# rasd3/TODA

Measured on NVIDIA B200. Metric: frames/s voxelize+VoxelResBackBone8x fwd+bwd, higher is better.
Workload: dtype bf16

## Files before the change

### include/toda_b200.h

```cpp
#ifndef TODA_B200_H
#define TODA_B200_H

#include <stddef.h>
#include <stdint.h>

#ifdef __cplusplus
extern "C" {
#endif

#define TODA_OK 0
#define TODA_ERR_INVALID (-1)
#define TODA_ERR_CUDA (-2)
#define TODA_ERR_WORKSPACE (-3)
#define TODA_ERR_UNSUPPORTED (-4)

#define TODA_ORDER_FIRST_APPEARANCE 0
#define TODA_ORDER_CANONICAL 1

const char *toda_last_error(void);
int toda_version(void);
long long toda_launch_count(void);
int toda_device_info(int *sm_count_host, int *cc_major_host, int *cc_minor_host);

size_t toda_index_bytes(int batch, int D, int H, int W);
int toda_index_insert(void *index, int batch, int D, int H, int W, const int32_t *coords, int n, void *stream);
int toda_index_insert_strided(void *index_out, int batch, int oD, int oH, int oW, const int32_t *in_coords, int n_in,
                              const int *ksize_host, const int *stride_host, const int *pad_host, void *stream);
int toda_index_build(void *index, int batch, int D, int H, int W, int32_t *out_coords, int cap, int32_t *n_out,
                     void *stream);
int toda_index_rows(const void *index, int batch, int D, int H, int W, const int32_t *coords, int n, int32_t *rows,
                    void *stream);
int toda_index_release(void *index, int batch, int D, int H, int W, const int32_t *coords, int n, void *stream);

#define TODA_SELECT_RANGE_XY 0
#define TODA_SELECT_RECT_XY 1
#define TODA_SELECT_SECTOR 2
#define TODA_SELECT_BOXES 3
size_t toda_points_select_workspace_bytes(int n);
int toda_points_select(const float *points, int n, int stride, int x_col, const int32_t *frame_offsets, int batch, int mode,
                       const double *params_host, int invert, int add_batch_col, float *out, int32_t *out_offsets,
                       void *workspace, size_t workspace_bytes, void *stream);

#define TODA_WORLD_FLIP_X 0
#define TODA_WORLD_FLIP_Y 1
#define TODA_WORLD_ROTATE 2
#define TODA_WORLD_SCALE 3
int toda_points_world_transform(const float *points, int n, int stride, int x_col, const int32_t *frame_offsets, int batch,
                                int n_steps, const int *kinds_host, const float *params_host, float *out, void *stream);

size_t toda_voxelize_workspace_bytes(int64_t n_points, int batch, const int *grid_host, int max_points,
                                     int max_voxels);
int toda_voxelize_hard(const float *points, int64_t n_points, int point_stride, int xyz_col, int feat_col,
                       int num_features, const int32_t *frame_offsets, int batch, const float *range_host,
                       const float *vsize_host, const int *grid_host, int max_points, int max_voxels, int order,
                       float *voxels, int32_t *coords, int32_t *num_points, int32_t *voxel_counts, void *workspace,
                       size_t workspace_bytes, void *stream);

int toda_mean_vfe_fwd(const float *voxels, const void *num_points, int num_is_float, int n_voxels, int max_points,
                      int num_features, float *voxel_features, void *stream);
int toda_mean_vfe_bwd(const float *d_voxel_features, const void *num_points, int num_is_float, int n_voxels,
                      int max_points, int num_features, float *d_voxels, void *stream);

int toda_rulebook_subm(const void *index, int batch, int D, int H, int W, const int32_t *coords, int n,
                       const int *ksize_host, int32_t *nbr, void *stream);
int toda_rulebook_sparse(const void *index_in, int iD, int iH, int iW, const void *index_out, int oD, int oH, int oW,
                         int batch, const int32_t *in_coords, int n_in, const int32_t *out_coords, int n_out,
                         const int *ksize_host, const int *stride_host, const int *pad_host, int32_t *nbr_fwd,
                         int32_t *nbr_bwd, void *stream);

size_t toda_parity_order_workspace_bytes(int n);
int toda_parity_order(const int32_t *coords, int n, const int *stride_host, const int *pad_host, int32_t *order,
                      int32_t *pos_of_row, void *workspace, size_t workspace_bytes, void *stream);

#define TODA_CONV_FP32 0
#define TODA_CONV_BF16 1
#define TODA_CONV_BF16X3 2
int toda_weight_repack(const float *w_param, int kvol, int cin, int cout, int transpose, int mirror_k, float *w_out,
                       void *stream);
size_t toda_spconv_fwd_workspace_bytes(int n_in, int cin, int cout, int kvol, int precision);
int toda_table_tile_masks(const int32_t *nbr, int n_out, int kvol, uint32_t *masks, void *stream);
int toda_spconv_uses_tensor_cores(int cin, int cout, int kvol, int precision);
int toda_spconv_wgrad_uses_tensor_cores(int cin, int cout, int kvol, int precision);
int toda_spconv_fwd(const float *x, const void *x_bf16, int n_in, int cin, const int32_t *nbr, int n_out, int kvol,
                    const float *w, int cout, const float *bias, float *y, const int32_t *out_rows,
                    const uint32_t *tile_masks, double *bn_sums, int precision, void *workspace, size_t workspace_bytes,
                    void *stream);
int toda_tile_plan_capacity(int channels);
int toda_table_tile_plan(const int32_t *nbr, int n_out, int kvol, int ngroups, int cap, uint16_t *lidx, int32_t *rows,
                         int32_t *cnt, void *stream);
int toda_spconv_fwd_plan(const float *x, const void *x_bf16, int n_in, int cin, const int32_t *nbr, int n_out, int kvol,
                         const float *w, int cout, const float *bias, const float *addend, float *y,
                         const int32_t *out_rows, const uint32_t *tile_masks, const uint16_t *plan_lidx,
                         const int32_t *plan_rows, const int32_t *plan_cnt, int plan_groups, int plan_cap, double *bn_sums,
                         const void *w_bf16, int precision, void *workspace, size_t workspace_bytes, void *stream);
int toda_weight_kmajor_bf16(const float *w, int kvol, int cin, int cout, void *w_bf16, void *stream);
size_t toda_spconv_wgrad_workspace_bytes(int n_in, int n_out, int kvol, int cin, int cout, int precision);
int toda_spconv_wgrad(const float *x, const void *x_bf16, int n_in, int cin, const int32_t *nbr, int n_out, int kvol,
                      const uint32_t *tile_masks, const float *dy, const void *dy_bf16, int cout, float *dw_param,
                      void *workspace, size_t workspace_bytes, int precision, void *stream);
int toda_spconv_wgrad_row_splits(const uint32_t *tile_masks, int n_out, int kvol, int cin, int cout, int *groups,
                                 int *splits, int32_t *row_begin, void *stream);

size_t toda_bn_workspace_bytes(int channels);
int toda_bn_local_sums(const float *y, const double *epilogue_sums, int n, int channels, double *sums, double *count,
                       void *workspace, size_t workspace_bytes, void *stream);
int toda_bn_eval_coeffs(const float *gamma, const float *beta, const float *running_mean, const float *running_var,
                        float eps, int channels, float *scale, float *shift, void *stream);
int toda_bn_apply(const float *y, int n, int channels, const float *scale, const float *shift, const float *residual,
                  int relu, float *a, void *a_bf16, void *stream);
int toda_bn_apply_sums(const float *y, int n, int channels, const double *sums, const double *count, const float *gamma,
                       const float *beta, float eps, float momentum, float *running_mean, float *running_var, float *scale,
                       float *shift, float *save_mean, float *save_rstd, const float *residual, int relu, float *a,
                       void *a_bf16, void *stream);
int toda_bn_bwd_reduce(const float *da, const float *a, const float *y, int n, int channels, const float *save_mean,
                       const float *save_rstd, int relu, double *red, float *dgamma, float *dbeta, void *workspace,
                       size_t workspace_bytes, void *stream);
int toda_bn_bwd_finish(const float *da, const float *a, const float *y, int n, int channels, const float *gamma,
                       const float *save_mean, const float *save_rstd, int relu, int training, const double *red,
                       const double *count, float *dy, void *dy_bf16, float *dresidual, float *dbias, void *workspace,
                       size_t workspace_bytes, void *stream);
int toda_bn_bwd(const float *da, const float *a, const float *y, int n, int channels, const float *gamma,
                const float *save_mean, const float *save_rstd, int relu, int training, float *dy, void *dy_bf16,
                float *dresidual, float *dgamma, float *dbeta, float *dbias, void *workspace, size_t workspace_bytes,
                void *stream);
int toda_col_sum(const float *dy, int n, int channels, float *out, void *workspace, size_t workspace_bytes,
                 void *stream);

typedef struct {
    const float *x; const void *x_bf16; int n_in, cin; const int32_t *nbr; int n_out, kvol;
    const float *w; const void *w_bf16 ; int cout; const float *bias ;
    const uint32_t *tile_masks ;
    const uint16_t *plan_lidx ; const int32_t *plan_rows; const int32_t *plan_cnt; int plan_groups, plan_cap;
    int precision; void *conv_ws; size_t conv_ws_bytes;
    const float *gamma; const float *beta; float eps, momentum; float *running_mean; float *running_var; int training;
    const float *residual ; int relu;
    float *y; double *sums; float *stats; float *a; void *a_bf16 ;
    void *bn_ws; size_t bn_ws_bytes;
} toda_layer_fwd_args;
typedef struct {
    const float *da; const float *a_mask; const float *y; int n_out, cout; const float *gamma; const float *mean; const float *rstd;
    int relu, training; float *dy; void *dy_bf16 ; float *dres ; float *dgamma; float *dbeta;
    void *bn_ws; size_t bn_ws_bytes;
    const float *x; const void *x_bf16 ; int n_in, cin, kvol;
    int need_dx; const int32_t *dgrad_nbr; const float *wt; const void *wt_bf16 ;
    const int32_t *dgrad_out_rows ; const uint32_t *dgrad_masks ;
    const uint16_t *dplan_lidx ; const int32_t *dplan_rows; const int32_t *dplan_cnt; int dplan_groups, dplan_cap;
    const float *addend ; float *dx;
    int need_dw; const int32_t *nbr_fwd; const uint32_t *fwd_masks ; float *dw;
    void *wgrad_ws; size_t wgrad_ws_bytes;
    int need_db; float *db;
    int precision; void *conv_ws; size_t conv_ws_bytes;
} toda_layer_bwd_args;
int toda_layer_fwd(const toda_layer_fwd_args *args, void *stream);
int toda_layer_bwd(const toda_layer_bwd_args *args, void *stream);
int toda_layer_fwd_stats(const toda_layer_fwd_args *args, double *local_sums, void *stream);
int toda_layer_fwd_apply(const toda_layer_fwd_args *args, const double *global_sums, void *stream);
int toda_layer_bwd_reduce(const toda_layer_bwd_args *args, double *local_red, void *stream);
int toda_layer_bwd_finish(const toda_layer_bwd_args *args, const double *global_red, const double *global_count, void *stream);

int toda_bev_scatter_fwd(const float *features, const int32_t *coords, int n, int channels, int batch, int D, int H,
                         int W, float *out, void *stream);
int toda_bev_scatter_bwd(const float *d_out, const int32_t *coords, int n, int channels, int batch, int D, int H,
                         int W, float *d_features, void *stream);

int toda_gather_rows(const float *in, const int32_t *rows, int n, int channels, float *out, void *stream);

#ifdef __cplusplus
}
#endif
#endif
```

### toda_b200/_C.py

```python
import ctypes
import os

_HERE = os.path.dirname(os.path.abspath(__file__))
LIB_PATH = os.path.join(_HERE, "lib", "libtoda_b200.so")

c_int, c_i64, c_f32, c_vp, c_sz = ctypes.c_int, ctypes.c_int64, ctypes.c_float, ctypes.c_void_p, ctypes.c_size_t
_IP = ctypes.POINTER(ctypes.c_int)
_FP = ctypes.POINTER(ctypes.c_float)

SIGNATURES = {
    "toda_last_error": (ctypes.c_char_p, []),
    "toda_version": (c_int, []),
    "toda_launch_count": (ctypes.c_longlong, []),
    "toda_device_info": (c_int, [_IP, _IP, _IP]),
    "toda_index_bytes": (c_sz, [c_int] * 4),
    "toda_index_insert": (c_int, [c_vp, c_int, c_int, c_int, c_int, c_vp, c_int, c_vp]),
    "toda_index_insert_strided": (c_int, [c_vp, c_int, c_int, c_int, c_int, c_vp, c_int, _IP, _IP, _IP, c_vp]),
    "toda_index_build": (c_int, [c_vp, c_int, c_int, c_int, c_int, c_vp, c_int, c_vp, c_vp]),
    "toda_index_rows": (c_int, [c_vp, c_int, c_int, c_int, c_int, c_vp, c_int, c_vp, c_vp]),
    "toda_index_release": (c_int, [c_vp, c_int, c_int, c_int, c_int, c_vp, c_int, c_vp]),
    "toda_points_select_workspace_bytes": (c_sz, [c_int]),
    "toda_points_select": (c_int, [c_vp, c_int, c_int, c_int, c_vp, c_int, c_int, ctypes.POINTER(ctypes.c_double), c_int, c_int,
                                   c_vp, c_vp, c_vp, c_sz, c_vp]),
    "toda_points_world_transform": (c_int, [c_vp, c_int, c_int, c_int, c_vp, c_int, c_int, _IP, _FP, c_vp, c_vp]),
    "toda_voxelize_workspace_bytes": (c_sz, [c_i64, c_int, _IP, c_int, c_int]),
    "toda_voxelize_hard": (c_int, [c_vp, c_i64, c_int, c_int, c_int, c_int, c_vp, c_int, _FP, _FP, _IP, c_int, c_int,
                                   c_int, c_vp, c_vp, c_vp, c_vp, c_vp, c_sz, c_vp]),
    "toda_mean_vfe_fwd": (c_int, [c_vp, c_vp, c_int, c_int, c_int, c_int, c_vp, c_vp]),
    "toda_mean_vfe_bwd": (c_int, [c_vp, c_vp, c_int, c_int, c_int, c_int, c_vp, c_vp]),
    "toda_rulebook_subm": (c_int, [c_vp, c_int, c_int, c_int, c_int, c_vp, c_int, _IP, c_vp, c_vp]),
    "toda_rulebook_sparse": (c_int, [c_vp, c_int, c_int, c_int, c_vp, c_int, c_int, c_int, c_int, c_vp, c_int, c_vp,
                                     c_int, _IP, _IP, _IP, c_vp, c_vp, c_vp]),
    "toda_weight_repack": (c_int, [c_vp, c_int, c_int, c_int, c_int, c_int, c_vp, c_vp]),
    "toda_spconv_fwd_workspace_bytes": (c_sz, [c_int] * 5),
    "toda_spconv_uses_tensor_cores": (c_int, [c_int] * 4),
    "toda_spconv_wgrad_uses_tensor_cores": (c_int, [c_int] * 4),
    "toda_parity_order_workspace_bytes": (c_sz, [c_int]),
    "toda_parity_order": (c_int, [c_vp, c_int, _IP, _IP, c_vp, c_vp, c_vp, c_sz, c_vp]),
    "toda_table_tile_masks": (c_int, [c_vp, c_int, c_int, c_vp, c_vp]),
    "toda_spconv_fwd": (c_int, [c_vp, c_vp, c_int, c_int, c_vp, c_int, c_int, c_vp, c_int, c_vp, c_vp, c_vp, c_vp, c_vp, c_int, c_vp,
                                c_sz, c_vp]),
    "toda_tile_plan_capacity": (c_int, [c_int]),
    "toda_table_tile_plan": (c_int, [c_vp, c_int, c_int, c_int, c_int, c_vp, c_vp, c_vp, c_vp]),
    "toda_spconv_fwd_plan": (c_int, [c_vp, c_vp, c_int, c_int, c_vp, c_int, c_int, c_vp, c_int, c_vp, c_vp, c_vp, c_vp, c_vp, c_vp,
                                     c_vp, c_vp, c_int, c_int, c_vp, c_vp, c_int, c_vp, c_sz, c_vp]),
    "toda_weight_kmajor_bf16": (c_int, [c_vp, c_int, c_int, c_int, c_vp, c_vp]),
    "toda_layer_fwd": (c_int, [c_vp, c_vp]),
    "toda_layer_bwd": (c_int, [c_vp, c_vp]),
    "toda_layer_fwd_stats": (c_int, [c_vp, c_vp, c_vp]),
    "toda_layer_fwd_apply": (c_int, [c_vp, c_vp, c_vp]),
    "toda_layer_bwd_reduce": (c_int, [c_vp, c_vp, c_vp]),
    "toda_layer_bwd_finish": (c_int, [c_vp, c_vp, c_vp, c_vp]),
    "toda_spconv_wgrad_workspace_bytes": (c_sz, [c_int] * 6),
    "toda_spconv_wgrad": (c_int, [c_vp, c_vp, c_int, c_int, c_vp, c_int, c_int, c_vp, c_vp, c_vp, c_int, c_vp, c_vp, c_sz, c_int,
                                  c_vp]),
    "toda_spconv_wgrad_row_splits": (c_int, [c_vp, c_int, c_int, c_int, c_int, _IP, _IP, c_vp, c_vp]),
    "toda_bn_workspace_bytes": (c_sz, [c_int]),
    "toda_bn_local_sums": (c_int, [c_vp, c_vp, c_int, c_int, c_vp, c_vp, c_vp, c_sz, c_vp]),
    "toda_bn_eval_coeffs": (c_int, [c_vp, c_vp, c_vp, c_vp, c_f32, c_int, c_vp, c_vp, c_vp]),
    "toda_bn_apply": (c_int, [c_vp, c_int, c_int, c_vp, c_vp, c_vp, c_int, c_vp, c_vp, c_vp]),
    "toda_bn_apply_sums": (c_int, [c_vp, c_int, c_int, c_vp, c_vp, c_vp, c_vp, c_f32, c_f32, c_vp, c_vp, c_vp, c_vp, c_vp, c_vp,
                                   c_vp, c_int, c_vp, c_vp, c_vp]),
    "toda_bn_bwd": (c_int, [c_vp, c_vp, c_vp, c_int, c_int, c_vp, c_vp, c_vp, c_int, c_int, c_vp, c_vp, c_vp, c_vp, c_vp,
                            c_vp, c_vp, c_sz, c_vp]),
    "toda_bn_bwd_reduce": (c_int, [c_vp, c_vp, c_vp, c_int, c_int, c_vp, c_vp, c_int, c_vp, c_vp, c_vp, c_vp, c_sz, c_vp]),
    "toda_bn_bwd_finish": (c_int, [c_vp, c_vp, c_vp, c_int, c_int, c_vp, c_vp, c_vp, c_int, c_int, c_vp, c_vp, c_vp, c_vp, c_vp,
                                   c_vp, c_vp, c_sz, c_vp]),
    "toda_col_sum": (c_int, [c_vp, c_int, c_int, c_vp, c_vp, c_sz, c_vp]),
    "toda_bev_scatter_fwd": (c_int, [c_vp, c_vp, c_int, c_int, c_int, c_int, c_int, c_int, c_vp, c_vp]),
    "toda_bev_scatter_bwd": (c_int, [c_vp, c_vp, c_int, c_int, c_int, c_int, c_int, c_int, c_vp, c_vp]),
    "toda_gather_rows": (c_int, [c_vp, c_vp, c_int, c_int, c_vp, c_vp]),
}



class LayerFwdArgs(ctypes.Structure):
    _fields_ = [("x", c_vp), ("x_bf16", c_vp), ("n_in", c_int), ("cin", c_int), ("nbr", c_vp), ("n_out", c_int), ("kvol", c_int),
                ("w", c_vp), ("w_bf16", c_vp), ("cout", c_int), ("bias", c_vp), ("tile_masks", c_vp),
                ("plan_lidx", c_vp), ("plan_rows", c_vp), ("plan_cnt", c_vp), ("plan_groups", c_int), ("plan_cap", c_int),
                ("precision", c_int), ("conv_ws", c_vp), ("conv_ws_bytes", c_sz),
                ("gamma", c_vp), ("beta", c_vp), ("eps", c_f32), ("momentum", c_f32), ("running_mean", c_vp), ("running_var", c_vp),
                ("training", c_int), ("residual", c_vp), ("relu", c_int),
                ("y", c_vp), ("sums", c_vp), ("stats", c_vp), ("a", c_vp), ("a_bf16", c_vp), ("bn_ws", c_vp), ("bn_ws_bytes", c_sz)]


class LayerBwdArgs(ctypes.Structure):
    _fields_ = [("da", c_vp), ("a_mask", c_vp), ("y", c_vp), ("n_out", c_int), ("cout", c_int), ("gamma", c_vp), ("mean", c_vp),
                ("rstd", c_vp), ("relu", c_int), ("training", c_int), ("dy", c_vp), ("dy_bf16", c_vp), ("dres", c_vp), ("dgamma", c_vp),
                ("dbeta", c_vp), ("bn_ws", c_vp), ("bn_ws_bytes", c_sz),
                ("x", c_vp), ("x_bf16", c_vp), ("n_in", c_int), ("cin", c_int), ("kvol", c_int),
                ("need_dx", c_int), ("dgrad_nbr", c_vp), ("wt", c_vp), ("wt_bf16", c_vp), ("dgrad_out_rows", c_vp), ("dgrad_masks", c_vp),
                ("dplan_lidx", c_vp), ("dplan_rows", c_vp), ("dplan_cnt", c_vp), ("dplan_groups", c_int), ("dplan_cap", c_int),
                ("addend", c_vp), ("dx", c_vp),
                ("need_dw", c_int), ("nbr_fwd", c_vp), ("fwd_masks", c_vp), ("dw", c_vp), ("wgrad_ws", c_vp), ("wgrad_ws_bytes", c_sz),
                ("need_db", c_int), ("db", c_vp),
                ("precision", c_int), ("conv_ws", c_vp), ("conv_ws_bytes", c_sz)]


_lib = None


def lib():
    global _lib
    if _lib is None:
        if not os.path.exists(LIB_PATH):
            raise RuntimeError(
                f"{LIB_PATH} is missing: build it with `python -c 'import __graft_entry__ as g; g.build()'` "
                "(nvcc, sm_100a).  toda_b200 has no CPU fallback.")
        L = ctypes.CDLL(LIB_PATH)
        for name, (res, args) in SIGNATURES.items():
            fn = getattr(L, name)
            fn.restype = res
            fn.argtypes = args
        _lib = L
    return _lib


def check(rc, what=""):
    if rc != 0:
        msg = lib().toda_last_error().decode("utf-8", "replace")
        raise RuntimeError(f"libtoda_b200 {what} failed (code {rc}): {msg}")


def ints(vals):
    return (ctypes.c_int * len(vals))(*[int(v) for v in vals])


def doubles(vals):
    return (ctypes.c_double * len(vals))(*[float(v) for v in vals])


def floats(vals):
    return (ctypes.c_float * len(vals))(*[float(v) for v in vals])
```

### toda_b200/csrc/bn.cu

```cuda
#include <cuda_bf16.h>

#include "common.cuh"

namespace {

constexpr int kThreads = 256;
constexpr int kPartials = 2 * kNumSMs;
constexpr int kApplyPartials = 2048 / kThreads * kNumSMs;

template <int MODE>
__global__ void __launch_bounds__(kThreads) col_reduce_vec_kernel(const float *__restrict__ p0, const float *__restrict__ p1,
                                                                  const float *__restrict__ p2, int n, int c,
                                                                  const float *__restrict__ mean, const float *__restrict__ rstd,
                                                                  int relu, double *__restrict__ partial) {
    __shared__ double s0[kThreads * 4], s1[kThreads * 4];
    const int tpr = c >> 2;
    const int rpi = kThreads / tpr;
    const int tx = threadIdx.x % tpr, ty = threadIdx.x / tpr;
    double a0[4] = {0, 0, 0, 0}, a1[4] = {0, 0, 0, 0};
    float4 m4 = make_float4(0, 0, 0, 0), r4 = make_float4(0, 0, 0, 0);
    if (MODE == 1) { m4 = __ldg((const float4 *)mean + tx); r4 = __ldg((const float4 *)rstd + tx); }
    const long long stride = (long long)gridDim.x * rpi;
    const bool active = ty < rpi;
    constexpr int U = 4;
    for (long long r = (long long)blockIdx.x * rpi + ty; active && r < n; r += U * stride) {
        float4 v0[U], v1[U], v2[U];
        bool ok[U];
#pragma unroll
        for (int u = 0; u < U; ++u) {
            long long rr = r + u * stride;
            ok[u] = rr < n;
            size_t e = ok[u] ? (size_t)rr * tpr + tx : 0;
            v0[u] = __ldg((const float4 *)p0 + e);
            if (MODE == 1) { v1[u] = __ldg((const float4 *)p1 + e); v2[u] = __ldg((const float4 *)p2 + e); }
        }
#pragma unroll
        for (int u = 0; u < U; ++u) {
            if (!ok[u]) continue;
            float x[4] = {v0[u].x, v0[u].y, v0[u].z, v0[u].w};
            if (MODE == 0) {
#pragma unroll
                for (int q = 0; q < 4; ++q) { a0[q] += x[q]; a1[q] += (double)x[q] * x[q]; }
            } else if (MODE == 1) {
                float av[4] = {v1[u].x, v1[u].y, v1[u].z, v1[u].w}, yv[4] = {v2[u].x, v2[u].y, v2[u].z, v2[u].w};
                float mm[4] = {m4.x, m4.y, m4.z, m4.w}, rs[4] = {r4.x, r4.y, r4.z, r4.w};
#pragma unroll
                for (int q = 0; q < 4; ++q) {
                    float g = (relu && !(av[q] > 0.f)) ? 0.f : x[q];
                    float xh = (yv[q] - mm[q]) * rs[q];
                    a0[q] += g; a1[q] += (double)g * xh;
                }
            } else {
#pragma unroll
                for (int q = 0; q < 4; ++q) a0[q] += x[q];
            }
        }
    }
#pragma unroll
    for (int q = 0; q < 4; ++q) { s0[threadIdx.x * 4 + q] = a0[q]; s1[threadIdx.x * 4 + q] = a1[q]; }
    __syncthreads();
    if ((int)threadIdx.x < c) {
        int ch = threadIdx.x, txx = ch >> 2, q = ch & 3;
        double t0 = 0.0, t1 = 0.0;
        for (int j = 0; j < rpi; ++j) { t0 += s0[(j * tpr + txx) * 4 + q]; t1 += s1[(j * tpr + txx) * 4 + q]; }
        partial[((size_t)blockIdx.x * 2 + 0) * c + ch] = t0;
        partial[((size_t)blockIdx.x * 2 + 1) * c + ch] = t1;
    }
}

template <int MODE>
__global__ void __launch_bounds__(kThreads) col_reduce_kernel(const float *__restrict__ p0, const float *__restrict__ p1,
                                                              const float *__restrict__ p2, int n, int c,
                                                              const float *__restrict__ mean, const float *__restrict__ rstd,
                                                              int relu, double *__restrict__ partial) {
    __shared__ double s0[kThreads], s1[kThreads];
    const int cpad = c <= 16 ? 16 : (c <= 32 ? 32 : (c <= 64 ? 64 : (c <= 128 ? 128 : 256)));
    const int rows_per_iter = kThreads / cpad;
    const int tx = threadIdx.x % cpad, ty = threadIdx.x / cpad;
    double a0 = 0.0, a1 = 0.0;
    float m = 0.f, rs = 0.f;
    if (MODE == 1 && tx < c) { m = mean[tx]; rs = rstd[tx]; }
    for (long long r = (long long)blockIdx.x * rows_per_iter + ty; r < n; r += (long long)gridDim.x * rows_per_iter) {
        if (tx < c) {
            size_t e = (size_t)r * c + tx;
            if (MODE == 0) {
                float v = __ldg(p0 + e);
                a0 += v; a1 += (double)v * v;
            } else if (MODE == 1) {
                float g = __ldg(p0 + e);
                if (relu && !(__ldg(p1 + e) > 0.f)) g = 0.f;
                float xh = (__ldg(p2 + e) - m) * rs;
                a0 += g; a1 += (double)g * xh;
            } else {
                a0 += __ldg(p0 + e);
            }
        }
    }
    s0[threadIdx.x] = a0; s1[threadIdx.x] = a1;
    __syncthreads();
    if (threadIdx.x < cpad && threadIdx.x < c) {
        double t0 = 0.0, t1 = 0.0;
        for (int j = 0; j < rows_per_iter; ++j) { t0 += s0[j * cpad + threadIdx.x]; t1 += s1[j * cpad + threadIdx.x]; }
        partial[((size_t)blockIdx.x * 2 + 0) * c + threadIdx.x] = t0;
        partial[((size_t)blockIdx.x * 2 + 1) * c + threadIdx.x] = t1;
    }
}

static bool vec_channels(int c) { return c % 4 == 0 && kThreads % (c / 4) == 0; }

template <int MODE>
static void launch_col_reduce(const float *p0, const float *p1, const float *p2, int n, int c, const float *mean,
                              const float *rstd, int relu, double *partial, cudaStream_t st) {
    if (vec_channels(c))
        col_reduce_vec_kernel<MODE><<<kPartials, kThreads, 0, st>>>(p0, p1, p2, n, c, mean, rstd, relu, partial);
    else
        col_reduce_kernel<MODE><<<kPartials, kThreads, 0, st>>>(p0, p1, p2, n, c, mean, rstd, relu, partial);
}

template <int MAX_BLOCKS = kPartials, int ROWS = 2>
__device__ __forceinline__ void warp_sum_partials(const double *__restrict__ partial, int nblocks, int c, int ch, double &s,
                                                  double &ss) {
    const int lane = threadIdx.x & 31;
    constexpr int kPerLane = (MAX_BLOCKS + 31) / 32;
    double va[kPerLane], vb[kPerLane];
#pragma unroll
    for (int i = 0; i < kPerLane; ++i) {
        const int j = lane + 32 * i;
        const bool ok = j < nblocks;
        va[i] = ok ? partial[((size_t)j * ROWS) * c + ch] : 0.0;
        vb[i] = ok && ROWS == 2 ? partial[((size_t)j * ROWS + 1) * c + ch] : 0.0;
    }
    double a = 0.0, b = 0.0;
#pragma unroll
    for (int i = 0; i < kPerLane; ++i) { a += va[i]; b += vb[i]; }
#pragma unroll
    for (int o = 16; o > 0; o >>= 1) { a += __shfl_xor_sync(0xffffffffu, a, o); b += __shfl_xor_sync(0xffffffffu, b, o); }
    s = a; ss = b;
}

__device__ __forceinline__ void bn_coeffs(double s, double ss, int n, float g, float bt, float eps, float &scale, float &shift,
                                          float &meanf, float &rstd, double &var) {
    const double mean = n > 0 ? s / n : 0.0;
    var = n > 0 ? ss / n - mean * mean : 0.0;
    if (var < 0.0) var = 0.0;
    rstd = (float)(1.0 / sqrt(var + (double)eps));
    meanf = (float)mean;
    scale = __fmul_rn(g, rstd);
    shift = __fsub_rn(bt, __fmul_rn(__fmul_rn(meanf, g), rstd));
}

__device__ __forceinline__ void bn_update_running(float *running_mean, float *running_var, int ch, float momentum, float meanf,
                                                  double var, int n) {
    if (running_mean) running_mean[ch] = __fadd_rn(__fmul_rn(1.f - momentum, running_mean[ch]), __fmul_rn(momentum, meanf));
    if (running_var) {
        const double unbiased = n > 1 ? var * n / (n - 1) : var;
        running_var[ch] = __fadd_rn(__fmul_rn(1.f - momentum, running_var[ch]), __fmul_rn(momentum, (float)unbiased));
    }
}

__global__ void bn_local_sums_kernel(const double *partial, int nblocks, const double *src, int n, int c, double *out,
                                     double *count) {
    if (count && blockIdx.x == 0 && threadIdx.x == 0) *count = (double)n;
    int ch = (blockIdx.x * blockDim.x + threadIdx.x) >> 5;
    if (ch >= c) return;
    double s = 0.0, ss = 0.0;
    if (partial) warp_sum_partials(partial, nblocks, c, ch, s, ss);
    else if (src) { s = src[ch]; ss = src[c + ch]; }
    if ((threadIdx.x & 31) != 0) return;
    out[ch] = s;
    out[c + ch] = ss;
}

__global__ void bn_eval_coeffs_kernel(const float *gamma, const float *beta, const float *rm, const float *rv, float eps,
                                      int c, float *scale, float *shift) {
    int ch = blockIdx.x * blockDim.x + threadIdx.x;
    if (ch >= c) return;
    float rstd = 1.0f / sqrtf(rv[ch] + eps);
    float g = gamma ? gamma[ch] : 1.f, bt = beta ? beta[ch] : 0.f;
    scale[ch] = g * rstd;
    shift[ch] = bt - rm[ch] * g * rstd;
}

__device__ __forceinline__ void store_bf16x4(__nv_bfloat16 *__restrict__ dst, long long e, float4 o) {
    __nv_bfloat162 lo = __floats2bfloat162_rn(o.x, o.y), hi = __floats2bfloat162_rn(o.z, o.w);
    uint2 pk;
    pk.x = *(uint32_t *)&lo;
    pk.y = *(uint32_t *)&hi;
    ((uint2 *)dst)[e] = pk;
}

struct BnCoeffs {
    const double *sums; const double *count; int n;
    const float *gamma, *beta; float eps, momentum;
    float *running_mean, *running_var, *scale, *shift, *save_mean, *save_rstd;
};

template <bool VEC>
__global__ void __launch_bounds__(kThreads) bn_apply_kernel(const float *__restrict__ y, long long total, int c, BnCoeffs k,
                                                            const float *__restrict__ residual, int relu, float *__restrict__ a,
                                                            __nv_bfloat16 *__restrict__ a_bf16) {
    extern __shared__ __align__(16) float s_coef[];
    float *s_sc = s_coef, *s_sh = s_coef + c;
    const int n = k.count ? (int)*k.count : k.n;
    for (int ch = threadIdx.x; ch < c; ch += blockDim.x) {
        if (!k.sums) {
            s_sc[ch] = k.scale[ch];
            s_sh[ch] = k.shift[ch];
            continue;
        }
        float meanf, rstd;
        double var;
        bn_coeffs(k.sums[ch], k.sums[c + ch], n, k.gamma ? k.gamma[ch] : 1.f, k.beta ? k.beta[ch] : 0.f, k.eps, s_sc[ch], s_sh[ch],
                  meanf, rstd, var);
        if (blockIdx.x == 0) {
            k.scale[ch] = s_sc[ch];
            k.shift[ch] = s_sh[ch];
            if (k.save_mean) k.save_mean[ch] = meanf;
            if (k.save_rstd) k.save_rstd[ch] = rstd;
            if (n > 0) bn_update_running(k.running_mean, k.running_var, ch, k.momentum, meanf, var, n);
        }
    }
    __syncthreads();
    const long long stride = (long long)gridDim.x * blockDim.x;
    long long e = blockIdx.x * (long long)blockDim.x + threadIdx.x;
    if (VEC) {
        const long long tv = total >> 2;
        const int ch = (int)((e << 2) % c);
        const float4 sc = *(const float4 *)(s_sc + ch), sh = *(const float4 *)(s_sh + ch);
        for (; e < tv; e += stride) {
            const float4 v = __ldg((const float4 *)y + e);
            float4 o = make_float4(fmaf(v.x, sc.x, sh.x), fmaf(v.y, sc.y, sh.y), fmaf(v.z, sc.z, sh.z), fmaf(v.w, sc.w, sh.w));
            if (residual) {
                const float4 r = __ldg((const float4 *)residual + e);
                o.x += r.x; o.y += r.y; o.z += r.z; o.w += r.w;
            }
            if (relu) { o.x = fmaxf(o.x, 0.f); o.y = fmaxf(o.y, 0.f); o.z = fmaxf(o.z, 0.f); o.w = fmaxf(o.w, 0.f); }
            ((float4 *)a)[e] = o;
            if (a_bf16) store_bf16x4(a_bf16, e, o);
        }
    } else {
        for (; e < total; e += stride) {
            const int ch = (int)(e % c);
            float o = fmaf(__ldg(y + e), s_sc[ch], s_sh[ch]);
            if (residual) o += __ldg(residual + e);
            if (relu) o = fmaxf(o, 0.f);
            a[e] = o;
            if (a_bf16) a_bf16[e] = __float2bfloat16_rn(o);
        }
    }
}

__global__ void bn_bwd_finalize_kernel(const double *__restrict__ partial, int nblocks, int c, float *dgamma, float *dbeta,
                                       double *sums) {
    int ch = (blockIdx.x * blockDim.x + threadIdx.x) >> 5;
    if (ch >= c) return;
    double s, sx;
    warp_sum_partials(partial, nblocks, c, ch, s, sx);
    if ((threadIdx.x & 31) != 0) return;
    if (dbeta) dbeta[ch] = (float)s;
    if (dgamma) dgamma[ch] = (float)sx;
    sums[ch] = s;
    sums[c + ch] = sx;
}

template <bool VEC>
__global__ void __launch_bounds__(kThreads, 5) bn_bwd_apply_kernel(const float *__restrict__ da, const float *__restrict__ a,
                                                                const float *__restrict__ y, long long total, int c, int n,
                                                                const double *__restrict__ count, const float *__restrict__ gamma,
                                                                const float *__restrict__ mean, const float *__restrict__ rstd,
                                                                const double *__restrict__ sums, int relu, int training,
                                                                float *__restrict__ dy, float *__restrict__ dres,
                                                                __nv_bfloat16 *__restrict__ dy_bf16, double *__restrict__ db_partial) {
    extern __shared__ double s_db[];
    double db[4] = {0.0, 0.0, 0.0, 0.0};
    if (count) n = (int)*count;
    auto sum = [&](int i) -> float { return (float)sums[i]; };
    const float inv_n = n > 0 ? 1.0f / (float)n : 0.f;
    const long long threads = (long long)gridDim.x * blockDim.x;
    const long long stride = VEC ? threads : threads / c * c;
    long long e = blockIdx.x * (long long)blockDim.x + threadIdx.x;
    if (VEC) {
        const long long tv = total >> 2;
        const int ch = (int)((e << 2) % c);
        float A[4], B[4], C[4];
#pragma unroll
        for (int q = 0; q < 4; ++q) {
            float gm = gamma ? gamma[ch + q] : 1.f, rs = rstd[ch + q];
            A[q] = gm * rs;
            B[q] = training ? -gm * rs * rs * sum(c + ch + q) * inv_n : 0.f;
            C[q] = training ? -A[q] * sum(ch + q) * inv_n - B[q] * mean[ch + q] : 0.f;
        }
        for (; e < tv; e += stride) {
            float4 g4 = __ldg((const float4 *)da + e);
            float4 y4 = training ? __ldg((const float4 *)y + e) : make_float4(0.f, 0.f, 0.f, 0.f);
            if (relu) {
                float4 a4 = __ldg((const float4 *)a + e);
                g4.x = a4.x > 0.f ? g4.x : 0.f; g4.y = a4.y > 0.f ? g4.y : 0.f;
                g4.z = a4.z > 0.f ? g4.z : 0.f; g4.w = a4.w > 0.f ? g4.w : 0.f;
            }
            if (dres) ((float4 *)dres)[e] = g4;
            float4 o;
            o.x = fmaf(A[0], g4.x, fmaf(B[0], y4.x, C[0]));
            o.y = fmaf(A[1], g4.y, fmaf(B[1], y4.y, C[1]));
            o.z = fmaf(A[2], g4.z, fmaf(B[2], y4.z, C[2]));
            o.w = fmaf(A[3], g4.w, fmaf(B[3], y4.w, C[3]));
            if (dy) ((float4 *)dy)[e] = o;
            if (dy_bf16) store_bf16x4(dy_bf16, e, o);
            if (db_partial) { db[0] += o.x; db[1] += o.y; db[2] += o.z; db[3] += o.w; }
        }
    } else {
        for (e = e < stride ? e : total; e < total; e += stride) {
            int ch = (int)(e % c);
            float g = __ldg(da + e);
            if (relu && !(__ldg(a + e) > 0.f)) g = 0.f;
            if (dres) dres[e] = g;
            float gm = gamma ? gamma[ch] : 1.f;
            float rs = rstd[ch];
            float o;
            if (training) {
                float xh = (__ldg(y + e) - mean[ch]) * rs;
                o = gm * rs * (g - sum(ch) * inv_n - xh * sum(c + ch) * inv_n);
            } else {
                o = gm * rs * g;
            }
            if (dy) dy[e] = o;
            if (dy_bf16) dy_bf16[e] = __float2bfloat16_rn(o);
            if (db_partial) db[0] += o;
        }
    }
    if (!db_partial) return;
    constexpr int kSlots = VEC ? 4 : 1;
#pragma unroll
    for (int q = 0; q < kSlots; ++q) s_db[threadIdx.x * kSlots + q] = db[q];
    __syncthreads();
    if ((int)threadIdx.x < c) {
        const int units = VEC ? c / 4 : c;
        const int u = VEC ? (int)threadIdx.x >> 2 : (int)threadIdx.x, q = VEC ? (int)threadIdx.x & 3 : 0;
        double t = 0.0;
        for (int j = u; j < kThreads; j += units) t += s_db[j * kSlots + q];
        const int ch = VEC ? (int)threadIdx.x : (int)(((long long)blockIdx.x * kThreads + threadIdx.x) % c);
        db_partial[(size_t)blockIdx.x * c + ch] = t;
    }
}

template <int MAX_BLOCKS, int ROWS>
__global__ void col_sum_finalize_kernel(const double *__restrict__ partial, int nblocks, int c, float *out) {
    int ch = (blockIdx.x * blockDim.x + threadIdx.x) >> 5;
    if (ch >= c) return;
    double s, unused;
    warp_sum_partials<MAX_BLOCKS, ROWS>(partial, nblocks, c, ch, s, unused);
    if ((threadIdx.x & 31) == 0) out[ch] = (float)s;
}

size_t partials_bytes(int c) {
    return (size_t)(2 * kPartials > kApplyPartials ? 2 * kPartials : kApplyPartials) * c * sizeof(double);
}
size_t bn_ws_bytes(int c) { return align_up(partials_bytes(c) + 2 * c * sizeof(double), 256); }

template <auto Kernel> int resident_grid(int64_t items) {
    static const int64_t cap = [] {
        int per_sm = 0;
        if (cudaOccupancyMaxActiveBlocksPerMultiprocessor(&per_sm, Kernel, kThreads, 0) != cudaSuccess || per_sm < 1) per_sm = 4;
        return (int64_t)per_sm * kNumSMs;
    }();
    const int64_t need = (items + kThreads - 1) / kThreads;
    return (int)(need < 1 ? 1 : (need < cap ? need : cap));
}

int launch_bn_apply(const float *y, int n, int c, const BnCoeffs &k, const float *residual, int relu, float *a, void *a_bf16,
                    cudaStream_t st) {
    const long long total = (long long)n * c;
    const size_t smem = 2 * (size_t)c * sizeof(float);
    if (vec_channels(c))
        bn_apply_kernel<true><<<resident_grid<bn_apply_kernel<true>>(total / 4), kThreads, smem, st>>>(
            y, total, c, k, residual, relu, a, (__nv_bfloat16 *)a_bf16);
    else
        bn_apply_kernel<false><<<resident_grid<bn_apply_kernel<false>>(total), kThreads, smem, st>>>(
            y, total, c, k, residual, relu, a, (__nv_bfloat16 *)a_bf16);
    TODA_LAUNCH_OK();
    return TODA_OK;
}

}

extern "C" size_t toda_bn_workspace_bytes(int channels) { return channels > 0 ? bn_ws_bytes(channels) : 0; }

double *bn_workspace_red(void *workspace, int c) { return (double *)((char *)workspace + partials_bytes(c)); }

extern "C" int toda_bn_local_sums(const float *y, const double *epilogue_sums, int n, int c, double *sums, double *count,
                                  void *workspace, size_t workspace_bytes, void *stream) {
    TODA_CHECK_ARG(n >= 0 && c > 0 && c <= 256 && sums, "bn_local_sums: bad args n=%d c=%d", n, c);
    if (n > 0 && epilogue_sums == sums && !count) return TODA_OK;
    cudaStream_t st = (cudaStream_t)stream;
    const double *partial = nullptr;
    if (n > 0 && !epilogue_sums) {
        TODA_CHECK_ARG(y && workspace, "bn_local_sums: null pointer");
        if (workspace_bytes < bn_ws_bytes(c)) { toda_set_error("bn_local_sums: workspace too small"); return TODA_ERR_WORKSPACE; }
        launch_col_reduce<0>(y, nullptr, nullptr, n, c, nullptr, nullptr, 0, (double *)workspace, st);
        TODA_LAUNCH_OK();
        partial = (const double *)workspace;
    }
    bn_local_sums_kernel<<<ceil_div(c * 32, 128), 128, 0, st>>>(partial, kPartials, n > 0 ? epilogue_sums : nullptr, n, c, sums,
                                                              count);
    TODA_LAUNCH_OK();
    return TODA_OK;
}

extern "C" int toda_bn_eval_coeffs(const float *gamma, const float *beta, const float *running_mean, const float *running_var,
                                   float eps, int c, float *scale, float *shift, void *stream) {
    TODA_CHECK_ARG(c > 0 && running_mean && running_var && scale && shift, "bn_eval_coeffs: bad args");
    bn_eval_coeffs_kernel<<<ceil_div(c, 128), 128, 0, (cudaStream_t)stream>>>(gamma, beta, running_mean, running_var, eps, c,
                                                                             scale, shift);
    TODA_LAUNCH_OK();
    return TODA_OK;
}

extern "C" int toda_bn_apply(const float *y, int n, int c, const float *scale, const float *shift, const float *residual,
                             int relu, float *a, void *a_bf16, void *stream) {
    TODA_CHECK_ARG(n >= 0 && c > 0, "bn_apply: bad sizes");
    if (n == 0) return TODA_OK;
    TODA_CHECK_ARG(y && scale && shift && a, "bn_apply: null pointer");
    BnCoeffs k{};
    k.scale = (float *)scale;
    k.shift = (float *)shift;
    return launch_bn_apply(y, n, c, k, residual, relu, a, a_bf16, (cudaStream_t)stream);
}

extern "C" int toda_bn_apply_sums(const float *y, int n, int c, const double *sums, const double *count, const float *gamma,
                                  const float *beta, float eps, float momentum, float *running_mean, float *running_var,
                                  float *scale, float *shift, float *save_mean, float *save_rstd, const float *residual, int relu,
                                  float *a, void *a_bf16, void *stream) {
    TODA_CHECK_ARG(n >= 0 && c > 0 && sums && scale && shift, "bn_apply_sums: bad args");
    TODA_CHECK_ARG(n == 0 || (y && a), "bn_apply_sums: null pointer");
    const BnCoeffs k{sums, count, n, gamma, beta, eps, momentum, running_mean, running_var, scale, shift, save_mean, save_rstd};
    return launch_bn_apply(y, n, c, k, residual, relu, a, a_bf16, (cudaStream_t)stream);
}

extern "C" int toda_bn_bwd_reduce(const float *da, const float *a, const float *y, int n, int c, const float *save_mean,
                                  const float *save_rstd, int relu, double *local_red, float *dgamma, float *dbeta, void *workspace,
                                  size_t workspace_bytes, void *stream) {
    TODA_CHECK_ARG(n >= 0 && c > 0 && c <= 256, "bn_bwd_reduce: unsupported sizes n=%d c=%d", n, c);
    TODA_CHECK_ARG(save_mean && save_rstd && workspace && local_red && (n == 0 || (da && y)) && (!relu || a || n == 0),
                   "bn_bwd_reduce: null pointer");
    if (workspace_bytes < bn_ws_bytes(c)) { toda_set_error("bn_bwd_reduce: workspace too small"); return TODA_ERR_WORKSPACE; }
    cudaStream_t st = (cudaStream_t)stream;
    double *partial = (double *)workspace;
    launch_col_reduce<1>(da, a, y, n, c, save_mean, save_rstd, relu, partial, st);
    TODA_LAUNCH_OK();
    bn_bwd_finalize_kernel<<<ceil_div(c * 32, 128), 128, 0, st>>>(partial, kPartials, c, dgamma, dbeta, local_red);
    TODA_LAUNCH_OK();
    return TODA_OK;
}

extern "C" int toda_bn_bwd_finish(const float *da, const float *a, const float *y, int n, int c, const float *gamma,
                                  const float *save_mean, const float *save_rstd, int relu, int training, const double *red,
                                  const double *count, float *dy, void *dy_bf16, float *dresidual, float *dbias, void *workspace,
                                  size_t workspace_bytes, void *stream) {
    TODA_CHECK_ARG(n >= 0 && c > 0 && c <= 256, "bn_bwd_finish: unsupported sizes n=%d c=%d", n, c);
    TODA_CHECK_ARG(save_mean && save_rstd && (red || !training) && (n == 0 || (da && y && (dy || dy_bf16))) &&
                   (!relu || a || n == 0) && (!dbias || workspace), "bn_bwd_finish: null pointer");
    cudaStream_t st = (cudaStream_t)stream;
    if (dbias && workspace_bytes < bn_ws_bytes(c)) { toda_set_error("bn_bwd_finish: workspace too small"); return TODA_ERR_WORKSPACE; }
    if (n == 0) {
        if (dbias) TODA_CUDA_OK(cudaMemsetAsync(dbias, 0, sizeof(float) * c, st));
        return TODA_OK;
    }
    const long long total = (long long)n * c;
    double *db_partial = dbias ? (double *)workspace : nullptr;
    const size_t smem = dbias ? kThreads * 4 * sizeof(double) : 0;
    int grid;
    if (vec_channels(c)) {
        grid = resident_grid<bn_bwd_apply_kernel<true>>(total / 4);
        grid = grid < kApplyPartials ? grid : kApplyPartials;
        bn_bwd_apply_kernel<true><<<grid, kThreads, smem, st>>>(da, a, y, total, c, n, count, gamma, save_mean, save_rstd, red, relu,
                                                               training, dy, dresidual, (__nv_bfloat16 *)dy_bf16, db_partial);
    } else {
        grid = resident_grid<bn_bwd_apply_kernel<false>>(total);
        grid = grid < kApplyPartials ? grid : kApplyPartials;
        bn_bwd_apply_kernel<false><<<grid, kThreads, smem, st>>>(da, a, y, total, c, n, count, gamma, save_mean, save_rstd, red,
                                                                relu, training, dy, dresidual, (__nv_bfloat16 *)dy_bf16, db_partial);
    }
    TODA_LAUNCH_OK();
    if (dbias) {
        col_sum_finalize_kernel<kApplyPartials, 1><<<ceil_div(c * 32, 128), 128, 0, st>>>(db_partial, grid, c, dbias);
        TODA_LAUNCH_OK();
    }
    return TODA_OK;
}

extern "C" int toda_bn_bwd(const float *da, const float *a, const float *y, int n, int c, const float *gamma,
                           const float *save_mean, const float *save_rstd, int relu, int training, float *dy, void *dy_bf16,
                           float *dresidual, float *dgamma, float *dbeta, float *dbias, void *workspace, size_t workspace_bytes,
                           void *stream) {
    TODA_CHECK_ARG(workspace, "bn_bwd: null workspace");
    double *red = bn_workspace_red(workspace, c);
    int rc = toda_bn_bwd_reduce(da, a, y, n, c, save_mean, save_rstd, relu, red, dgamma, dbeta, workspace, workspace_bytes, stream);
    if (rc) return rc;
    return toda_bn_bwd_finish(da, a, y, n, c, gamma, save_mean, save_rstd, relu, training, red, nullptr, dy, dy_bf16, dresidual,
                              dbias, workspace, workspace_bytes, stream);
}

extern "C" int toda_col_sum(const float *dy, int n, int c, float *out, void *workspace, size_t workspace_bytes, void *stream) {
    TODA_CHECK_ARG(n >= 0 && c > 0 && c <= 256 && out && workspace, "col_sum: bad args");
    if (workspace_bytes < bn_ws_bytes(c)) { toda_set_error("col_sum: workspace too small"); return TODA_ERR_WORKSPACE; }
    cudaStream_t st = (cudaStream_t)stream;
    double *partial = (double *)workspace;
    launch_col_reduce<2>(dy, nullptr, nullptr, n, c, nullptr, nullptr, 0, partial, st);
    TODA_LAUNCH_OK();
    col_sum_finalize_kernel<kPartials, 2><<<ceil_div(c * 32, 128), 128, 0, st>>>(partial, kPartials, c, out);
    TODA_LAUNCH_OK();
    return TODA_OK;
}
```

### toda_b200/csrc/layer.cu

```cuda
#include "common.cuh"

static int layer_conv(const toda_layer_fwd_args *p, double *bn_sums, void *stream) {
    return toda_spconv_fwd_plan(p->x, p->x_bf16, p->n_in, p->cin, p->nbr, p->n_out, p->kvol, p->w, p->cout, p->bias, nullptr, p->y,
                                nullptr, p->tile_masks, p->plan_lidx, p->plan_rows, p->plan_cnt, p->plan_groups, p->plan_cap,
                                bn_sums, p->w_bf16, p->precision, p->conv_ws, p->conv_ws_bytes, stream);
}

static int layer_fwd_stats(const toda_layer_fwd_args *p, double *sums, double *count, void *stream) {
    const int c = p->cout, n = p->n_out;
    const bool tc = n > 0 && toda_spconv_uses_tensor_cores(p->cin, c, p->kvol, p->precision);
    int rc = layer_conv(p, tc ? sums : nullptr, stream);
    if (rc) return rc;
    return toda_bn_local_sums(p->y, tc ? sums : nullptr, n, c, sums, count, p->bn_ws, p->bn_ws_bytes, stream);
}

static int layer_fwd_apply(const toda_layer_fwd_args *p, const double *sums, const double *count, void *stream) {
    const int c = p->cout;
    float *scale = p->stats, *shift = p->stats + c, *mean = p->stats + 2 * c, *rstd = p->stats + 3 * c;
    return toda_bn_apply_sums(p->y, p->n_out, c, sums, count, p->gamma, p->beta, p->eps, p->momentum, p->running_mean,
                              p->running_var, scale, shift, mean, rstd, p->residual, p->relu, p->a, p->a_bf16, stream);
}

extern "C" int toda_layer_fwd(const toda_layer_fwd_args *p, void *stream) {
    TODA_CHECK_ARG(p, "layer_fwd: null args");
    const int c = p->cout, n = p->n_out;
    TODA_CHECK_ARG(c > 0 && n >= 0 && p->stats && (n == 0 || (p->y && p->a)) && (!p->training || p->sums),
                   "layer_fwd: bad sizes / null outputs");
    if (n == 0) return layer_conv(p, nullptr, stream);
    int rc;
    if (p->training) {
        rc = layer_fwd_stats(p, p->sums, nullptr, stream);
        return rc ? rc : layer_fwd_apply(p, p->sums, nullptr, stream);
    }
    float *scale = p->stats, *shift = p->stats + c;
    if ((rc = layer_conv(p, nullptr, stream))) return rc;
    if ((rc = toda_bn_eval_coeffs(p->gamma, p->beta, p->running_mean, p->running_var, p->eps, c, scale, shift, stream))) return rc;
    return toda_bn_apply(p->y, n, c, scale, shift, p->residual, p->relu, p->a, p->a_bf16, stream);
}

static int layer_bwd_empty(const toda_layer_bwd_args *p, bool bn_grads, cudaStream_t st) {
    const int c = p->cout;
    if (bn_grads && p->dgamma) TODA_CUDA_OK(cudaMemsetAsync(p->dgamma, 0, sizeof(float) * c, st));
    if (bn_grads && p->dbeta) TODA_CUDA_OK(cudaMemsetAsync(p->dbeta, 0, sizeof(float) * c, st));
    if (p->need_db && p->db) TODA_CUDA_OK(cudaMemsetAsync(p->db, 0, sizeof(float) * c, st));
    if (p->need_dw && p->dw) TODA_CUDA_OK(cudaMemsetAsync(p->dw, 0, sizeof(float) * (size_t)p->kvol * p->cin * c, st));
    if (p->need_dx && p->dx && p->n_in > 0) {
        if (p->addend) TODA_CUDA_OK(cudaMemcpyAsync(p->dx, p->addend, sizeof(float) * (size_t)p->n_in * p->cin, cudaMemcpyDeviceToDevice, st));
        else TODA_CUDA_OK(cudaMemsetAsync(p->dx, 0, sizeof(float) * (size_t)p->n_in * p->cin, st));
    }
    return TODA_OK;
}

static bool layer_bwd_reads_dy_f32(const toda_layer_bwd_args *p) {
    const int c = p->cout;
    return !p->dy_bf16 || p->precision != TODA_CONV_BF16 ||
           (p->need_dx && !toda_spconv_uses_tensor_cores(c, p->cin, p->kvol, p->precision)) ||
           (p->need_dw && !toda_spconv_wgrad_uses_tensor_cores(p->cin, c, p->kvol, p->precision));
}

static int layer_bwd_conv(const toda_layer_bwd_args *p, void *stream) {
    const int c = p->cout, n = p->n_out;
    int rc;
    if (p->need_dx) {
        rc = toda_spconv_fwd_plan(p->dy, p->dy_bf16, n, c, p->dgrad_nbr, p->n_in, p->kvol, p->wt, p->cin, nullptr, p->addend, p->dx,
                                  p->dgrad_out_rows, p->dgrad_masks, p->dplan_lidx, p->dplan_rows, p->dplan_cnt, p->dplan_groups,
                                  p->dplan_cap, nullptr, p->wt_bf16, p->precision, p->conv_ws, p->conv_ws_bytes, stream);
        if (rc) return rc;
    }
    if (p->need_dw) {
        rc = toda_spconv_wgrad(p->x, p->x_bf16, p->n_in, p->cin, p->nbr_fwd, n, p->kvol, p->fwd_masks, p->dy, p->dy_bf16, c, p->dw,
                               p->wgrad_ws, p->wgrad_ws_bytes, p->precision, stream);
        if (rc) return rc;
    }
    return TODA_OK;
}

static int layer_bwd_reduce(const toda_layer_bwd_args *p, double *red, void *stream) {
    return toda_bn_bwd_reduce(p->da, p->a_mask, p->y, p->n_out, p->cout, p->mean, p->rstd, p->relu, red, p->dgamma, p->dbeta,
                              p->bn_ws, p->bn_ws_bytes, stream);
}

static int layer_bwd_finish(const toda_layer_bwd_args *p, const double *red, const double *count, void *stream) {
    const int c = p->cout, n = p->n_out;
    if (n == 0) return layer_bwd_empty(p, false, (cudaStream_t)stream);
    int rc = toda_bn_bwd_finish(p->da, p->a_mask, p->y, n, c, p->gamma, p->mean, p->rstd, p->relu, p->training, red, count,
                                layer_bwd_reads_dy_f32(p) ? p->dy : nullptr, p->dy_bf16, p->dres, p->need_db ? p->db : nullptr,
                                p->bn_ws, p->bn_ws_bytes, stream);
    return rc ? rc : layer_bwd_conv(p, stream);
}

extern "C" int toda_layer_bwd(const toda_layer_bwd_args *p, void *stream) {
    TODA_CHECK_ARG(p, "layer_bwd: null args");
    TODA_CHECK_ARG(p->cout > 0 && p->n_out >= 0, "layer_bwd: bad sizes");
    if (p->n_out == 0) return layer_bwd_empty(p, true, (cudaStream_t)stream);
    TODA_CHECK_ARG(p->bn_ws, "layer_bwd: null workspace");
    double *red = bn_workspace_red(p->bn_ws, p->cout);
    int rc = layer_bwd_reduce(p, red, stream);
    return rc ? rc : layer_bwd_finish(p, red, nullptr, stream);
}


extern "C" int toda_layer_fwd_stats(const toda_layer_fwd_args *p, double *local_sums, void *stream) {
    TODA_CHECK_ARG(p && local_sums, "layer_fwd_stats: null args");
    const int c = p->cout, n = p->n_out;
    TODA_CHECK_ARG(c > 0 && n >= 0 && p->training && (n == 0 || p->y), "layer_fwd_stats: bad sizes / not training / null y");
    return layer_fwd_stats(p, local_sums, local_sums + 2 * c, stream);
}

extern "C" int toda_layer_fwd_apply(const toda_layer_fwd_args *p, const double *global_sums, void *stream) {
    TODA_CHECK_ARG(p && global_sums, "layer_fwd_apply: null args");
    const int c = p->cout, n = p->n_out;
    TODA_CHECK_ARG(c > 0 && n >= 0 && p->training && p->stats && (n == 0 || (p->y && p->a)),
                   "layer_fwd_apply: bad sizes / not training / null outputs");
    return layer_fwd_apply(p, global_sums, global_sums + 2 * c, stream);
}

extern "C" int toda_layer_bwd_reduce(const toda_layer_bwd_args *p, double *local_red, void *stream) {
    TODA_CHECK_ARG(p && local_red, "layer_bwd_reduce: null args");
    TODA_CHECK_ARG(p->cout > 0 && p->n_out >= 0 && p->training, "layer_bwd_reduce: bad sizes / not training");
    return layer_bwd_reduce(p, local_red, stream);
}

extern "C" int toda_layer_bwd_finish(const toda_layer_bwd_args *p, const double *global_red, const double *global_count,
                                     void *stream) {
    TODA_CHECK_ARG(p && global_red && global_count, "layer_bwd_finish: null args");
    TODA_CHECK_ARG(p->cout > 0 && p->n_out >= 0 && p->training, "layer_bwd_finish: bad sizes / not training");
    return layer_bwd_finish(p, global_red, global_count, stream);
}
```

### toda_b200/ops.py

```python
import ctypes
import weakref
from dataclasses import dataclass
from typing import List, Optional

import numpy as np
import torch
import torch.distributed as dist

from . import _C

ORDER_FIRST_APPEARANCE = 0
ORDER_CANONICAL = 1
CONV_FP32 = 0
CONV_BF16 = 1
CONV_BF16X3 = 2
_TC_PRECISIONS = (CONV_BF16, CONV_BF16X3)

_launch_base = 0


def launches():
    return int(_C.lib().toda_launch_count()) - _launch_base


def reset_launches():
    global _launch_base
    _launch_base = int(_C.lib().toda_launch_count())



_prof = None


def profile_begin():
    global _prof
    _prof = []


def profile_end():
    global _prof
    rec, _prof = _prof, None
    torch.cuda.synchronize()
    return [dict(name=n, ms=a.elapsed_time(b), **m) for (n, m, a, b) in rec]


class _Timed:
    def __init__(self, name, meta):
        self.name, self.meta = name, meta

    def __enter__(self):
        self.a = torch.cuda.Event(enable_timing=True)
        self.a.record()
        return self

    def __exit__(self, *exc):
        b = torch.cuda.Event(enable_timing=True)
        b.record()
        _prof.append((self.name, self.meta, self.a, b))
        return False


class _NoTimer:
    def __enter__(self):
        return self

    def __exit__(self, *exc):
        return False


_NO_TIMER = _NoTimer()


def _timed(name, **meta):
    return _Timed(name, meta) if _prof is not None else _NO_TIMER


_raw_stream = torch._C._cuda_getCurrentRawStream


def _stream_id(device=None):
    return _raw_stream(torch.cuda.current_device() if device is None or device.index is None else device.index)


def _stream():
    return ctypes.c_void_p(_raw_stream(torch.cuda.current_device()))


def _p(t: Optional[torch.Tensor]):
    return ctypes.c_void_p(t.data_ptr()) if t is not None else None


def _need(t, dtype, name):
    if not t.is_cuda:
        raise RuntimeError(f"{name} must be a CUDA tensor (toda_b200 has no CPU path)")
    if t.dtype != dtype:
        raise TypeError(f"{name} must be {dtype}, got {t.dtype}")
    if not t.is_contiguous():
        raise ValueError(f"{name} must be contiguous")
    return t


_workspaces = {}


def _workspace(tag, nbytes, device, zero=False):
    key = (tag, device.index, _stream_id(device))
    buf = _workspaces.get(key)
    if buf is None or buf.numel() < nbytes:
        buf = (torch.zeros if zero else torch.empty)(int(nbytes * 1.25) + 256, dtype=torch.uint8, device=device)
        _workspaces[key] = buf
    return buf


SELECT_RANGE_XY, SELECT_RECT_XY, SELECT_SECTOR, SELECT_BOXES = 0, 1, 2, 3
SELECT_MAX_BOXES = 96


def points_select(points, frame_offsets, mode, params, invert=False, add_batch_col=False, x_col=0, trim=True):
    points = _need(points, torch.float32, "points")
    assert points.dim() == 2
    n, stride = points.shape
    dev = points.device
    batch = 0
    if frame_offsets is not None:
        frame_offsets = _need(frame_offsets, torch.int32, "frame_offsets")
        batch = frame_offsets.numel() - 1
    L = _C.lib()
    ws = _workspace("select", L.toda_points_select_workspace_bytes(n), dev)
    out = torch.empty((n, stride + (1 if add_batch_col else 0)), dtype=torch.float32, device=dev)
    out_offsets = torch.empty((batch + 1,), dtype=torch.int32, device=dev)
    p = list(params) + [0.0] * (4 - len(params))
    with _timed("points_select", n=n, stride=stride, mode=int(mode)):
        _C.check(L.toda_points_select(_p(points), n, stride, int(x_col), _p(frame_offsets), batch, int(mode), _C.doubles(p),
                                      int(bool(invert)), int(bool(add_batch_col)), _p(out), _p(out_offsets), _p(ws),
                                      ws.numel(), _stream()), "toda_points_select")
    if trim:
        return out[:int(out_offsets[-1].item())], out_offsets
    return out, out_offsets


WORLD_FLIP_X, WORLD_FLIP_Y, WORLD_ROTATE, WORLD_SCALE = 0, 1, 2, 3
WORLD_MAX_STEPS = 4
WORLD_MAX_BATCH = 64


def points_world_transform(points, frame_offsets, steps, x_col=0):
    points = _need(points, torch.float32, "points")
    if points.dim() != 2:
        raise ValueError("points must be (N, stride)")
    n, stride = points.shape
    if not (0 <= x_col and x_col + 2 < stride <= 63):
        raise ValueError(f"points_world_transform: x, y, z at columns {x_col}..{x_col + 2} do not fit stride {stride} (<= 63)")
    batch = 1
    if frame_offsets is not None:
        frame_offsets = _need(frame_offsets, torch.int32, "frame_offsets")
        batch = frame_offsets.numel() - 1
        if not 1 <= batch <= WORLD_MAX_BATCH:
            raise ValueError(f"points_world_transform: batch {batch} outside [1, {WORLD_MAX_BATCH}]")
    if len(steps) > WORLD_MAX_STEPS:
        raise ValueError(f"points_world_transform: {len(steps)} steps (at most {WORLD_MAX_STEPS})")
    kinds, params = [], np.zeros((len(steps), batch, 2), np.float32)
    for s, (kind, values) in enumerate(steps):
        if kind not in (WORLD_FLIP_X, WORLD_FLIP_Y, WORLD_ROTATE, WORLD_SCALE):
            raise ValueError(f"points_world_transform: unknown step kind {kind!r}")
        v = np.asarray(values, dtype=np.float32).reshape(batch, -1)
        if v.shape[1] != (2 if kind == WORLD_ROTATE else 1):
            raise ValueError(f"points_world_transform: step {s} needs {2 if kind == WORLD_ROTATE else 1} value(s) per frame for "
                             f"{batch} frame(s), got {np.shape(values)}")
        kinds.append(int(kind))
        params[s, :, :v.shape[1]] = v
    out = torch.empty_like(points)
    with _timed("points_world_transform", n=n, stride=stride, steps=len(steps)):
        _C.check(_C.lib().toda_points_world_transform(_p(points), n, stride, int(x_col), _p(frame_offsets), batch, len(kinds),
                                                      _C.ints(kinds or [0]), _C.floats(params.reshape(-1).tolist() or [0.0]),
                                                      _p(out), _stream()), "toda_points_world_transform")
    return out


def gather_point_rows(points, rows):
    points = _need(points, torch.float32, "points")
    rows = _need(rows, torch.int32, "rows")
    n, c = rows.shape[0], points.shape[1]
    out = torch.empty((n, c), dtype=torch.float32, device=points.device)
    _C.check(_C.lib().toda_gather_rows(_p(points), _p(rows), n, c, _p(out), _stream()), "toda_gather_rows")
    return out


def grid_size_xyz(pc_range, voxel_size):
    r = np.asarray(pc_range, dtype=np.float64)
    return np.round((r[3:6] - r[0:3]) / np.asarray(voxel_size, dtype=np.float64)).astype(np.int64)


def voxelize(points, frame_offsets, pc_range, voxel_size, max_points, max_voxels, num_features=None, xyz_col=0,
             feat_col=0, order=ORDER_FIRST_APPEARANCE, grid=None, trim=True):
    points = _need(points, torch.float32, "points")
    assert points.dim() == 2
    n, stride = points.shape
    dev = points.device
    if not torch.is_tensor(frame_offsets):
        frame_offsets = torch.tensor(list(frame_offsets), dtype=torch.int32, device=dev)
    frame_offsets = _need(frame_offsets, torch.int32, "frame_offsets")
    batch = frame_offsets.numel() - 1
    f = int(num_features) if num_features is not None else stride - feat_col
    grid = grid_size_xyz(pc_range, voxel_size) if grid is None else np.asarray(grid)
    grid_c = _C.ints(grid)
    L = _C.lib()
    ws_bytes = L.toda_voxelize_workspace_bytes(n, batch, grid_c, max_points, max_voxels)
    if ws_bytes == 0:
        raise RuntimeError("toda_voxelize_workspace_bytes rejected the arguments")
    ws = _workspace("vox", ws_bytes, dev)
    cap = batch * max_voxels
    voxels = torch.empty((cap, max_points, f), dtype=torch.float32, device=dev)
    coords = torch.empty((cap, 4), dtype=torch.int32, device=dev)
    num = torch.empty((cap,), dtype=torch.int32, device=dev)
    counts = torch.empty((batch + 1,), dtype=torch.int32, device=dev)
    with _timed("voxelize", n_points=n, batch=batch, K=max_points, F=f):
        rc = L.toda_voxelize_hard(_p(points), n, stride, xyz_col, feat_col, f, _p(frame_offsets), batch,
                                  _C.floats(np.asarray(pc_range, dtype=np.float32)),
                                  _C.floats(np.asarray(voxel_size, dtype=np.float32)), grid_c, max_points, max_voxels,
                                  order, _p(voxels), _p(coords), _p(num), _p(counts), _p(ws), ws.numel(), _stream())
    _C.check(rc, "toda_voxelize_hard")
    if trim:
        v = int(counts[batch].item())
        return voxels[:v], coords[:v], num[:v], counts
    return voxels, coords, num, counts


class _MeanVFE(torch.autograd.Function):
    @staticmethod
    def forward(ctx, voxels, num_points):
        voxels = _need(voxels, torch.float32, "voxels")
        v, k, f = voxels.shape
        is_float = num_points.dtype == torch.float32
        if not is_float:
            num_points = _need(num_points, torch.int32, "voxel_num_points")
        num_points = num_points.contiguous()
        out = torch.empty((v, f), dtype=torch.float32, device=voxels.device)
        with _timed("mean_vfe_fwd", V=v, K=k, F=f):
            _C.check(_C.lib().toda_mean_vfe_fwd(_p(voxels), _p(num_points), int(is_float), v, k, f, _p(out), _stream()),
                     "toda_mean_vfe_fwd")
        ctx.save_for_backward(num_points)
        ctx.shape = (v, k, f, is_float)
        return out

    @staticmethod
    def backward(ctx, dout):
        (num_points,) = ctx.saved_tensors
        v, k, f, is_float = ctx.shape
        dout = dout.contiguous()
        dv = torch.empty((v, k, f), dtype=torch.float32, device=dout.device)
        _C.check(_C.lib().toda_mean_vfe_bwd(_p(dout), _p(num_points), int(is_float), v, k, f, _p(dv), _stream()),
                 "toda_mean_vfe_bwd")
        return dv, None


def mean_vfe(voxels, num_points):
    return _MeanVFE.apply(voxels, num_points)


_index_occupant = {}


class OccupancyIndex:

    def __init__(self, batch, shape, device, tag):
        self.batch = int(batch)
        self.shape = [int(s) for s in shape]
        d, h, w = self.shape
        nbytes = _C.lib().toda_index_bytes(self.batch, d, h, w)
        if nbytes == 0:
            raise RuntimeError(f"bad index dims {batch} {shape}")
        self.key = (("index", tag, self.batch, d, h, w), device.index, _stream_id(device))
        self.buf = _workspace(self.key[0], nbytes, device, zero=True)
        self.coords = None
        self.frame_counts = None
        self.n = 0
        self._marked = False

    def _dims(self):
        return (self.batch, *self.shape)

    def _acquire(self):
        prev = _index_occupant.get(self.key)
        if prev is not None and prev is not self and prev.buf.data_ptr() == self.buf.data_ptr():
            prev._unmark()
        _index_occupant[self.key] = self

    def _unmark(self):
        if self.coords is not None and self.n > 0:
            _C.check(_C.lib().toda_index_release(_p(self.buf), *self._dims(), _p(self.coords), self.n, _stream()),
                     "toda_index_release")
        if _index_occupant.get(self.key) is self:
            del _index_occupant[self.key]

    def insert(self, coords):
        self._acquire()
        coords = _need(coords, torch.int32, "coords")
        _C.check(_C.lib().toda_index_insert(_p(self.buf), *self._dims(), _p(coords), coords.shape[0], _stream()),
                 "toda_index_insert")

    def insert_strided(self, in_coords, ksize, stride, padding):
        self._acquire()
        in_coords = _need(in_coords, torch.int32, "in_coords")
        _C.check(_C.lib().toda_index_insert_strided(_p(self.buf), *self._dims(), _p(in_coords), in_coords.shape[0],
                                                    _C.ints(ksize), _C.ints(stride), _C.ints(padding), _stream()),
                 "toda_index_insert_strided")

    def build(self, cap, known_n=None):
        dev = self.buf.device
        coords = torch.empty((max(cap, 1), 4), dtype=torch.int32, device=dev)
        n_out = torch.empty((self.batch + 1,), dtype=torch.int32, device=dev)
        with _timed("index_build", cells=self.batch * self.shape[0] * self.shape[1] * self.shape[2]):
            _C.check(_C.lib().toda_index_build(_p(self.buf), *self._dims(), _p(coords), cap, _p(n_out), _stream()),
                     "toda_index_build")
        self.n = int(n_out[0].item()) if known_n is None else int(known_n)
        self.coords = coords[:self.n]
        self.frame_counts = n_out
        return self.coords

    def ensure_live(self):
        if _index_occupant.get(self.key) is self:
            return
        if self.coords is None:
            raise RuntimeError("occupancy index was released")
        coords, n = self.coords, self.n
        self.insert(coords)
        self.build(n, known_n=n)

    def rows(self, coords):
        self.ensure_live()
        coords = _need(coords, torch.int32, "coords")
        rows = torch.empty((coords.shape[0],), dtype=torch.int32, device=coords.device)
        _C.check(_C.lib().toda_index_rows(_p(self.buf), *self._dims(), _p(coords), coords.shape[0], _p(rows), _stream()),
                 "toda_index_rows")
        return rows

    def release(self):
        if _index_occupant.get(self.key) is self:
            self._unmark()
        self.coords = None
        self.n = 0


@dataclass
class Rulebook:
    subm: bool
    ksize: List[int]
    stride: List[int]
    padding: List[int]
    in_shape: List[int]
    out_shape: List[int]
    n_in: int
    n_out: int
    out_coords: torch.Tensor
    nbr_fwd: torch.Tensor
    nbr_bwd: Optional[torch.Tensor]
    dgrad_order: Optional[torch.Tensor] = None
    nbr_bwd_sorted: Optional[torch.Tensor] = None
    dgrad_tile_masks: Optional[torch.Tensor] = None
    tile_masks: Optional[torch.Tensor] = None
    plan: Optional["TilePlan"] = None
    dgrad_plan: Optional["TilePlan"] = None

    @property
    def kvol(self):
        return self.ksize[0] * self.ksize[1] * self.ksize[2]


@dataclass
class TilePlan:
    lidx: torch.Tensor
    rows: torch.Tensor
    cnt: torch.Tensor
    ngroups: int
    cap: int

    def tensors(self):
        return [self.lidx, self.rows, self.cnt]


def table_tile_plan(nbr, ksize, channels):
    kvol, n = nbr.shape
    ngroups = int(ksize[0])
    if n == 0 or kvol > 27 or ngroups > 3 or kvol % ngroups or kvol // ngroups > 9 or not channels:
        return None
    L = _C.lib()
    cap = L.toda_tile_plan_capacity(int(channels))
    if cap <= 0:
        return None
    tiles = (n + 127) // 128
    dev = nbr.device
    lidx = torch.empty((tiles, kvol, 128), dtype=torch.int16, device=dev)
    rows = torch.empty((tiles, ngroups, cap), dtype=torch.int32, device=dev)
    cnt = torch.empty((tiles, ngroups), dtype=torch.int32, device=dev)
    with _timed("tile_plan", n=n, kvol=kvol):
        _C.check(L.toda_table_tile_plan(_p(nbr), n, kvol, ngroups, cap, _p(lidx), _p(rows), _p(cnt), _stream()),
                 "toda_table_tile_plan")
    return TilePlan(lidx, rows, cnt, ngroups, cap)


def conv_out_size(in_size, k, s, p):
    return (in_size + 2 * p - (k - 1) - 1) // s + 1


def rulebook_subm(index: OccupancyIndex, ksize, channels=None):
    index.ensure_live()
    n = index.n
    kvol = ksize[0] * ksize[1] * ksize[2]
    nbr = torch.empty((kvol, n), dtype=torch.int32, device=index.buf.device)
    with _timed("rulebook_subm", n=n, kvol=kvol):
        _C.check(_C.lib().toda_rulebook_subm(_p(index.buf), index.batch, *index.shape, _p(index.coords), n, _C.ints(ksize),
                                             _p(nbr), _stream()), "toda_rulebook_subm")
    rb = Rulebook(True, list(ksize), [1, 1, 1], [k // 2 for k in ksize], index.shape, index.shape, n, n, index.coords,
                  nbr, None)
    rb.tile_masks = table_tile_masks(nbr) if (n > 0 and kvol <= 32) else None
    rb.plan = table_tile_plan(nbr, ksize, channels) if _TILE_PLANS else None
    return rb


def rulebook_sparse(index_in: OccupancyIndex, ksize, stride, padding, tag, cin=None, cout=None):
    index_in.ensure_live()
    out_shape = [conv_out_size(index_in.shape[a], ksize[a], stride[a], padding[a]) for a in range(3)]
    index_out = OccupancyIndex(index_in.batch, out_shape, index_in.buf.device, tag)
    if index_out.buf.data_ptr() == index_in.buf.data_ptr():
        index_out = OccupancyIndex(index_in.batch, out_shape, index_in.buf.device, (tag, "alt"))
    assert index_out.buf.data_ptr() != index_in.buf.data_ptr()
    index_out.insert_strided(index_in.coords, ksize, stride, padding)
    per_in = 1
    for a in range(3):
        per_in *= min(ksize[a], (ksize[a] + stride[a] - 1) // stride[a])
    cells = index_in.batch * out_shape[0] * out_shape[1] * out_shape[2]
    cap = int(min(index_in.n * per_in, cells))
    out_coords = index_out.build(cap)
    n_in, n_out = index_in.n, index_out.n
    kvol = ksize[0] * ksize[1] * ksize[2]
    dev = index_in.buf.device
    nbr_fwd = torch.empty((kvol, n_out), dtype=torch.int32, device=dev)
    nbr_bwd = torch.empty((kvol, n_in), dtype=torch.int32, device=dev)
    with _timed("rulebook_sparse", n_in=n_in, n_out=n_out, kvol=kvol):
        _C.check(_C.lib().toda_rulebook_sparse(_p(index_in.buf), *index_in.shape, _p(index_out.buf), *out_shape,
                                               index_in.batch, _p(index_in.coords), n_in, _p(out_coords), n_out,
                                               _C.ints(ksize), _C.ints(stride), _C.ints(padding), _p(nbr_fwd), _p(nbr_bwd),
                                               _stream()), "toda_rulebook_sparse")
    rb = Rulebook(False, list(ksize), list(stride), list(padding), index_in.shape, out_shape, n_in, n_out, out_coords,
                  nbr_fwd, nbr_bwd)
    rb.tile_masks = table_tile_masks(nbr_fwd) if (n_out > 0 and kvol <= 32) else None
    rb.dgrad_order, rb.nbr_bwd_sorted = (_dgrad_parity_order(index_in.coords, nbr_bwd, stride, padding) if kvol <= 32
                                         else (None, None))
    if rb.dgrad_order is not None:
        rb.dgrad_tile_masks = table_tile_masks(rb.nbr_bwd_sorted)
    if _TILE_PLANS:
        rb.plan = table_tile_plan(nbr_fwd, ksize, cin)
        rb.dgrad_plan = table_tile_plan(rb.nbr_bwd_sorted if rb.dgrad_order is not None else nbr_bwd, ksize, cout)
    return rb, index_out


import os as _os
_TILE_PLANS = _os.environ.get("TODA_TILE_PLANS", "0") == "1"


def set_tile_plans(on):
    global _TILE_PLANS
    _TILE_PLANS = bool(on)


def tile_plans_enabled():
    return _TILE_PLANS


def table_tile_masks(nbr):
    kvol, n = nbr.shape
    masks = torch.empty(((n + 127) // 128,), dtype=torch.int32, device=nbr.device)
    _C.check(_C.lib().toda_table_tile_masks(_p(nbr), n, kvol, _p(masks), _stream()), "toda_table_tile_masks")
    return masks


def _dgrad_parity_order(in_coords, nbr_bwd, stride, padding):
    if all(s == 1 for s in stride) or in_coords.shape[0] == 0:
        return None, None
    if stride[0] * stride[1] * stride[2] > 8:
        return None, None
    n = in_coords.shape[0]
    L = _C.lib()
    ws = _workspace("parity", L.toda_parity_order_workspace_bytes(n), in_coords.device)
    order = torch.empty((n,), dtype=torch.int32, device=in_coords.device)
    _C.check(L.toda_parity_order(_p(in_coords), n, _C.ints(stride), _C.ints(padding), _p(order), None, _p(ws), ws.numel(),
                                 _stream()), "toda_parity_order")
    return order, nbr_bwd.index_select(1, order).contiguous()


_repack_cache = {}


def invalidate_weight_cache():
    _repack_cache.clear()


def _repack(weight, transpose, mirror, want_bf16=False):
    key = (id(weight), bool(transpose), bool(mirror))
    hit = _repack_cache.get(key)
    if hit is not None and hit[2]() is weight and hit[0] == weight._version and hit[3] == weight.data_ptr():
        out = hit[1]
    else:
        cout, kvol, cin = weight.shape[0], weight.shape[1] * weight.shape[2] * weight.shape[3], weight.shape[4]
        out = torch.empty((kvol, cout, cin) if transpose else (kvol, cin, cout), dtype=torch.float32, device=weight.device)
        _C.check(_C.lib().toda_weight_repack(_p(weight), kvol, cin, cout, int(transpose), int(mirror), _p(out), _stream()),
                 "toda_weight_repack")
        if len(_repack_cache) > 512:
            _repack_cache.clear()
        hit = [weight._version, out, weakref.ref(weight), weight.data_ptr(), None]
        _repack_cache[key] = hit
    if not want_bf16:
        return out
    if hit[4] is None:
        kvol, ci, co = out.shape
        wb = torch.empty((co, kvol * max(ci, 16)), dtype=torch.bfloat16, device=out.device)
        _C.check(_C.lib().toda_weight_kmajor_bf16(_p(out), kvol, ci, co, _p(wb), _stream()), "toda_weight_kmajor_bf16")
        hit[4] = wb
    return out, hit[4]


def _bf16_shadow_of(t):
    tag = getattr(t, "_toda_bf16", None)
    if tag is not None and tag[1] == t._version and tag[0].shape == t.shape:
        return tag[0]
    return None


def _conv_call(x, xb, cin, nbr, n_out, kvol, w, cout, bias, precision, what="conv_fwd", rb=None, bn_sums=None, y=None,
               out_rows=None, tile_masks=None, plan=None, addend=None, w_bf16=None):
    if y is None:
        y = torch.empty((n_out, cout), dtype=torch.float32, device=x.device)
    L = _C.lib()
    ws_bytes = L.toda_spconv_fwd_workspace_bytes(x.shape[0], cin, cout, kvol, precision)
    ws = _workspace("conv", ws_bytes, x.device) if ws_bytes else None
    if precision not in _TC_PRECISIONS:
        plan = None
    with _timed(what, n_in=x.shape[0], n_out=n_out, cin=cin, cout=cout, kvol=kvol, precision=precision, rb=id(rb)):
        if plan is None and addend is None and w_bf16 is None:
            _C.check(L.toda_spconv_fwd(_p(x), _p(xb), x.shape[0], cin, _p(nbr), n_out, kvol, _p(w), cout, _p(bias), _p(y),
                                       _p(out_rows), _p(tile_masks), _p(bn_sums), precision, _p(ws), ws.numel() if ws is not None else 0,
                                       _stream()), "toda_spconv_fwd")
        else:
            pl = plan
            _C.check(L.toda_spconv_fwd_plan(_p(x), _p(xb), x.shape[0], cin, _p(nbr), n_out, kvol, _p(w), cout, _p(bias),
                                            _p(addend), _p(y), _p(out_rows), _p(tile_masks), _p(pl.lidx) if pl else None,
                                            _p(pl.rows) if pl else None, _p(pl.cnt) if pl else None, pl.ngroups if pl else 0,
                                            pl.cap if pl else 0, _p(bn_sums), _p(w_bf16), precision, _p(ws),
                                            ws.numel() if ws is not None else 0, _stream()), "toda_spconv_fwd_plan")
    return y


def conv_plan_usable(plan, cin, cout, kvol, precision):
    if plan is None or precision not in _TC_PRECISIONS or _os.environ.get("TODA_TC_FEED", "ts")[:1] in ("c",) or \
            _os.environ.get("TODA_TC_FEED", "ts")[:2] == "tm":
        return False
    cp = max(16, cin)
    return (cp in (16, 32, 64, 128) and cout in (16, 32, 64, 128) and kvol <= 27
            and plan.cap <= _C.lib().toda_tile_plan_capacity(cp))


def _conv_forward_impl(x, x_bf16, weight, bias, rb, precision, want_stats):
    x = _need(x.contiguous(), torch.float32, "features")
    weight = _need(weight.contiguous(), torch.float32, "weight")
    cout, cin = weight.shape[0], weight.shape[4]
    assert x.shape == (rb.n_in, cin), (x.shape, rb.n_in, cin)
    if x_bf16 is not None and (precision != CONV_BF16 or x_bf16.shape != x.shape or x_bf16.dtype != torch.bfloat16
                               or not x_bf16.is_contiguous()):
        x_bf16 = None
    w = _repack(weight, False, False)
    b = bias.contiguous() if bias is not None else None
    sums = None
    if want_stats and rb.n_out > 0 and _C.lib().toda_spconv_uses_tensor_cores(cin, cout, rb.kvol, precision):
        sums = torch.empty((2 * cout,), dtype=torch.float64, device=x.device)
    y = _conv_call(x, x_bf16, cin, rb.nbr_fwd, rb.n_out, rb.kvol, w, cout, b, precision, "conv_fwd", rb, sums,
                   tile_masks=rb.tile_masks, plan=rb.plan)
    return y, sums, x, weight, x_bf16


def _conv_backward_impl(dy, dyb, x, weight, xb, rb, precision, need_dx, need_dw, need_db):
    cout, cin = weight.shape[0], weight.shape[4]
    L = _C.lib()
    dx = dw = db = None
    if need_dx:
        wt = _repack(weight, True, rb.subm)
        if rb.subm:
            dx = _conv_call(dy, dyb, cout, rb.nbr_fwd, rb.n_in, rb.kvol, wt, cin, None, precision, "conv_dgrad", rb,
                            tile_masks=rb.tile_masks, plan=rb.plan)
        elif rb.dgrad_order is None:
            dx = _conv_call(dy, dyb, cout, rb.nbr_bwd, rb.n_in, rb.kvol, wt, cin, None, precision, "conv_dgrad", rb,
                            plan=rb.dgrad_plan)
        else:
            dx = _conv_call(dy, dyb, cout, rb.nbr_bwd_sorted, rb.n_in, rb.kvol, wt, cin, None, precision, "conv_dgrad",
                            rb, out_rows=rb.dgrad_order, tile_masks=rb.dgrad_tile_masks, plan=rb.dgrad_plan)
    if need_dw:
        dw = torch.empty_like(weight)
        ws_bytes = L.toda_spconv_wgrad_workspace_bytes(rb.n_in, rb.n_out, rb.kvol, cin, cout, precision)
        ws = _workspace("wgrad", ws_bytes, dy.device)
        with _timed("conv_wgrad", n_in=rb.n_in, n_out=rb.n_out, cin=cin, cout=cout, kvol=rb.kvol, precision=precision,
                    rb=id(rb)):
            _C.check(L.toda_spconv_wgrad(_p(x), _p(xb), rb.n_in, cin, _p(rb.nbr_fwd), rb.n_out, rb.kvol, _p(rb.tile_masks),
                                         _p(dy), _p(dyb), cout, _p(dw), _p(ws), ws.numel(), precision, _stream()),
                     "toda_spconv_wgrad")
    if need_db:
        db = col_sum(dy)
    return dx, dw, db


class _SparseConv(torch.autograd.Function):
    @staticmethod
    def forward(ctx, x, x_bf16, weight, bias, rb: Rulebook, precision, want_stats):
        y, sums, x, weight, x_bf16 = _conv_forward_impl(x, x_bf16, weight, bias, rb, precision, want_stats)
        ctx.save_for_backward(x, weight, x_bf16)
        ctx.set_materialize_grads(False)
        ctx.rb, ctx.precision, ctx.has_bias = rb, precision, bias is not None
        if sums is not None:
            ctx.mark_non_differentiable(sums)
        return y, sums

    @staticmethod
    def backward(ctx, dy, _dsums=None):
        if dy is None:
            return (None,) * 7
        x, weight, xb = ctx.saved_tensors
        dyb = _bf16_shadow_of(dy) if (ctx.precision == CONV_BF16 and dy.is_contiguous()) else None
        dx, dw, db = _conv_backward_impl(dy.contiguous(), dyb, x, weight, xb, ctx.rb, ctx.precision, ctx.needs_input_grad[0],
                                         ctx.needs_input_grad[2], ctx.has_bias and ctx.needs_input_grad[3])
        return dx, None, dw, db, None, None, None


def sparse_conv(x, weight, bias, rb, precision=CONV_FP32, x_bf16=None, want_stats=False):
    y, sums = _SparseConv.apply(x, x_bf16, weight, bias, rb, precision, want_stats)
    return (y, sums) if want_stats else y


def col_sum(t):
    n, c = t.shape
    out = torch.empty((c,), dtype=torch.float32, device=t.device)
    L = _C.lib()
    ws = _workspace("bn", L.toda_bn_workspace_bytes(c), t.device)
    _C.check(L.toda_col_sum(_p(t), n, c, _p(out), _p(ws), ws.numel(), _stream()), "toda_col_sum")
    return out


class ReluMaskTape:

    def __init__(self, mode):
        assert mode in ("record", "replay")
        self.mode, self.masks, self.i = mode, [], 0

    def replay(self):
        self.mode, self.i = "replay", 0
        return self


_relu_tape = None


def set_relu_mask_tape(tape):
    global _relu_tape
    _relu_tape = tape


def sync_group(bn):
    if not isinstance(bn, torch.nn.SyncBatchNorm) or not bn.training:
        return None
    if bn.momentum is None:
        raise NotImplementedError("toda_b200: SyncBatchNorm with momentum=None (cumulative moving average) is not supported; "
                                  "set a momentum (these backbones use 0.01)")
    if not (dist.is_available() and dist.is_initialized()):
        return None
    group = bn.process_group if bn.process_group is not None else dist.group.WORLD
    return group if dist.get_world_size(group) > 1 else None


def _run_phases(phases, group):
    try:
        buf = next(phases)
        while True:
            dist.all_reduce(buf, op=dist.ReduceOp.SUM, group=group)
            buf = phases.send(None)
    except StopIteration as stop:
        return stop.value


def _tape_mask(a, want_bf16):
    if _relu_tape.mode == "record":
        mask = a > 0
        _relu_tape.masks.append(mask)
    else:
        mask = _relu_tape.masks[_relu_tape.i]
        _relu_tape.i += 1
    a = a * mask
    return a, (a.to(torch.bfloat16) if want_bf16 else None), mask.to(torch.float32)


def _bn_forward_phases(y, gamma, beta, running_mean, running_var, eps, momentum, training, residual, relu, want_bf16, sums,
                       need_grad, sync=False):
    y = _need(y.contiguous(), torch.float32, "bn input")
    n, c = y.shape
    dev = y.device
    L = _C.lib()
    scale, shift, mean, rstd = torch.empty((4, c), dtype=torch.float32, device=dev).unbind(0)
    gsums = count = None
    if training:
        if sync or sums is None:
            buf = torch.empty((2 * c + 1 if sync else 2 * c,), dtype=torch.float64, device=dev)
            count = buf.data_ptr() + 16 * c if sync else None
            ws = _workspace("bn", L.toda_bn_workspace_bytes(c), dev)
            with _timed("bn_stats", n=n, c=c):
                _C.check(L.toda_bn_local_sums(_p(y), _p(sums), n, c, _p(buf), count, _p(ws), ws.numel(), _stream()),
                         "toda_bn_local_sums")
            sums = buf
        if sync:
            yield sums
            gsums = sums
    else:
        _C.check(L.toda_bn_eval_coeffs(_p(gamma), _p(beta), _p(running_mean), _p(running_var), float(eps), c, _p(scale),
                                       _p(shift), _stream()), "toda_bn_eval_coeffs")
        mean = running_mean
        rstd = torch.rsqrt(running_var + eps) if need_grad else None
    res = residual.contiguous() if residual is not None else None
    a = torch.empty_like(y)
    tape = _relu_tape is not None and relu
    ab = torch.empty(y.shape, dtype=torch.bfloat16, device=dev) if (want_bf16 and not tape) else None
    act = 0 if tape else int(relu)
    with _timed("bn_apply", n=n, c=c, residual=res is not None):
        if training:
            _C.check(L.toda_bn_apply_sums(_p(y), n, c, _p(sums), count, _p(gamma), _p(beta), float(eps), float(momentum),
                                          _p(running_mean), _p(running_var), _p(scale), _p(shift), _p(mean), _p(rstd), _p(res),
                                          act, _p(a), _p(ab), _stream()), "toda_bn_apply_sums")
        else:
            _C.check(L.toda_bn_apply(_p(y), n, c, _p(scale), _p(shift), _p(res), act, _p(a), _p(ab), _stream()), "toda_bn_apply")
    if tape:
        a, ab, mask = _tape_mask(a, want_bf16)
        return a, ab, y, mean, rstd, mask, gsums
    return a, ab, y, mean, rstd, a, gsums


def _bn_backward_phases(da, y, a, gamma, mean, rstd, training, relu, has_res, want_bf16, gsums=None, want_db=False):
    n, c = y.shape
    da = da.contiguous() if da is not None else torch.zeros_like(y)
    L = _C.lib()
    dy = torch.empty_like(y)
    dyb = torch.empty(y.shape, dtype=torch.bfloat16, device=y.device) if want_bf16 else None
    dres = torch.empty_like(y) if has_res else None
    dgamma, dbeta = torch.empty((2, c), dtype=torch.float32, device=y.device).unbind(0)
    db = torch.empty((c,), dtype=torch.float32, device=y.device) if want_db else None
    ws = _workspace("bn", L.toda_bn_workspace_bytes(c), y.device)
    if gsums is None:
        with _timed("bn_bwd", n=n, c=c, residual=has_res):
            _C.check(L.toda_bn_bwd(_p(da), _p(a), _p(y), n, c, _p(gamma), _p(mean), _p(rstd), int(relu), int(training),
                                   _p(dy), _p(dyb), _p(dres), _p(dgamma), _p(dbeta), _p(db), _p(ws), ws.numel(), _stream()),
                     "toda_bn_bwd")
        return dy, dyb, dres, dgamma, dbeta, db
    red = torch.empty((2 * c,), dtype=torch.float64, device=y.device)
    _C.check(L.toda_bn_bwd_reduce(_p(da), _p(a), _p(y), n, c, _p(mean), _p(rstd), int(relu), _p(red), _p(dgamma), _p(dbeta),
                                  _p(ws), ws.numel(), _stream()), "toda_bn_bwd_reduce")
    yield red
    _C.check(L.toda_bn_bwd_finish(_p(da), _p(a), _p(y), n, c, _p(gamma), _p(mean), _p(rstd), int(relu), 1, _p(red),
                                  gsums.data_ptr() + 16 * c, _p(dy), _p(dyb), _p(dres), _p(db), _p(ws), ws.numel(), _stream()),
             "toda_bn_bwd_finish")
    return dy, dyb, dres, dgamma, dbeta, db


class _BNAct(torch.autograd.Function):
    @staticmethod
    def forward(ctx, y, gamma, beta, running_mean, running_var, eps, momentum, training, residual, relu, want_bf16, sums, group):
        a, ab, y, mean, rstd, a_mask, gsums = _run_phases(
            _bn_forward_phases(y, gamma, beta, running_mean, running_var, eps, momentum, training, residual, relu, want_bf16, sums,
                        y.requires_grad or gamma.requires_grad, group is not None), group)
        ctx.save_for_backward(y, a_mask, gamma, mean, rstd, gsums)
        ctx.set_materialize_grads(False)
        ctx.cfg = (bool(training), bool(relu), residual is not None, bool(want_bf16))
        ctx.group = group
        if ab is not None:
            ctx.mark_non_differentiable(ab)
        return a, ab

    @staticmethod
    def backward(ctx, da, _dab=None):
        if da is None and ctx.group is None:
            return (None,) * 13
        y, a, gamma, mean, rstd, gsums = ctx.saved_tensors
        training, relu, has_res, want_bf16 = ctx.cfg
        dy, dyb, dres, dgamma, dbeta, _ = _run_phases(_bn_backward_phases(da, y, a, gamma, mean, rstd, training, relu, has_res,
                                                                          want_bf16, gsums), ctx.group)
        if dyb is not None:
            dy._toda_bf16 = (dyb, dy._version)
        return dy, dgamma, dbeta, None, None, None, None, None, dres, None, None, None, None


def _vp(t):
    return t.data_ptr() if t is not None else None


def _fused_ok(training, need_grad):
    return _prof is None and _relu_tape is None and (training or not need_grad)


def _layer_forward(x, x_bf16, weight, bias, rb, precision, gamma, beta, running_mean, running_var, eps, momentum, training,
                   residual, relu, want_bf16, need_grad=True, group=None):
    return _run_phases(_layer_forward_phases(x, x_bf16, weight, bias, rb, precision, gamma, beta, running_mean, running_var, eps,
                                             momentum, residual, relu, want_bf16, need_grad, training, group is not None), group)


def _layer_forward_phases(x, x_bf16, weight, bias, rb, precision, gamma, beta, running_mean, running_var, eps, momentum,
                          residual, relu, want_bf16, need_grad=True, training=True, sync=True):
    if not _fused_ok(training, need_grad):
        y, sums, x, weight, x_bf16 = _conv_forward_impl(x, x_bf16, weight, bias, rb, precision, bool(training))
        a, ab, y, mean, rstd, a_mask, gsums = yield from _bn_forward_phases(y, gamma, beta, running_mean, running_var, eps,
                                                                            momentum, training, residual, relu, want_bf16, sums,
                                                                            need_grad, sync)
        return a, ab, (x, x_bf16, weight, y, a_mask, gamma, mean, rstd, gsums)
    args, x, x_bf16, weight, y, a, ab, small, _keep = _layer_fwd_args(
        x, x_bf16, weight, bias, rb, precision, gamma, beta, running_mean, running_var, eps, momentum, training, residual, relu,
        want_bf16)
    cout = y.shape[1]
    L = _C.lib()
    gsums = None
    if sync:
        gsums = torch.empty((2 * cout + 1,), dtype=torch.float64, device=y.device)
        _C.check(L.toda_layer_fwd_stats(ctypes.byref(args), _p(gsums), _stream()), "toda_layer_fwd_stats")
        yield gsums
        _C.check(L.toda_layer_fwd_apply(ctypes.byref(args), _p(gsums), _stream()), "toda_layer_fwd_apply")
    else:
        _C.check(L.toda_layer_fwd(ctypes.byref(args), _stream()), "toda_layer_fwd")
    mean = small[2 * cout:3 * cout] if training else running_mean
    rstd = small[3 * cout:4 * cout] if training else None
    return a, ab, (x, x_bf16, weight, y, a, gamma, mean, rstd, gsums)


def _layer_fwd_args(x, x_bf16, weight, bias, rb, precision, gamma, beta, running_mean, running_var, eps, momentum, training,
                    residual, relu, want_bf16):
    x = _need(x.contiguous(), torch.float32, "features")
    weight = _need(weight.contiguous(), torch.float32, "weight")
    cout, cin = weight.shape[0], weight.shape[4]
    assert x.shape == (rb.n_in, cin), (x.shape, rb.n_in, cin)
    if x_bf16 is not None and (precision != CONV_BF16 or x_bf16.shape != x.shape or x_bf16.dtype != torch.bfloat16
                               or not x_bf16.is_contiguous()):
        x_bf16 = None
    L = _C.lib()
    kvol, n_out, dev = rb.kvol, rb.n_out, x.device
    tc = bool(L.toda_spconv_uses_tensor_cores(cin, cout, kvol, precision))
    if tc and precision == CONV_BF16:
        w, wb = _repack(weight, False, False, True)
    else:
        w, wb = _repack(weight, False, False), None
    y = torch.empty((n_out, cout), dtype=torch.float32, device=dev)
    a = torch.empty_like(y)
    ab = torch.empty((n_out, cout), dtype=torch.bfloat16, device=dev) if want_bf16 else None
    small = torch.empty((8 * cout,), dtype=torch.float32, device=dev)
    ws_bytes = L.toda_spconv_fwd_workspace_bytes(x.shape[0], cin, cout, kvol, precision)
    ws = _workspace("conv", ws_bytes, dev) if ws_bytes else None
    bws = _workspace("bn", L.toda_bn_workspace_bytes(cout), dev)
    res = residual.contiguous() if residual is not None else None
    b = bias.contiguous() if bias is not None else None
    pl = rb.plan if precision in _TC_PRECISIONS else None
    sp = small.data_ptr()
    args = _C.LayerFwdArgs(
        x.data_ptr(), _vp(x_bf16), x.shape[0], cin, rb.nbr_fwd.data_ptr(), n_out, kvol, w.data_ptr(), _vp(wb), cout, _vp(b),
        _vp(rb.tile_masks), _vp(pl.lidx) if pl else None, _vp(pl.rows) if pl else None, _vp(pl.cnt) if pl else None,
        pl.ngroups if pl else 0, pl.cap if pl else 0, precision, _vp(ws), ws.numel() if ws is not None else 0,
        gamma.data_ptr(), beta.data_ptr(), float(eps), float(momentum), _vp(running_mean), _vp(running_var), int(bool(training)),
        _vp(res), int(bool(relu)), y.data_ptr(), sp + 16 * cout, sp, a.data_ptr(), _vp(ab), bws.data_ptr(), bws.numel())
    return args, x, x_bf16, weight, y, a, ab, small, (w, wb, ws, bws, res, b)


def _layer_backward(da, saved, rb, precision, training, relu, has_res, has_bias, need_dx, need_dw, addend=None, group=None):
    return _run_phases(_layer_backward_phases(da, saved, rb, precision, relu, has_res, has_bias, need_dx, need_dw, addend,
                                              training), group)


def _layer_backward_phases(da, saved, rb, precision, relu, has_res, has_bias, need_dx, need_dw, addend=None, training=True):
    x, xb, weight, y, a_mask, gamma, mean, rstd, gsums = saved
    if da is None:
        da = torch.zeros_like(y)
    if not _fused_ok(training, True):
        dy, dyb, dres, dgamma, dbeta, db = yield from _bn_backward_phases(da, y, a_mask, gamma, mean, rstd, training, relu,
                                                                          has_res, precision == CONV_BF16, gsums, has_bias)
        dx, dw, _ = _conv_backward_impl(dy, dyb, x, weight, xb, rb, precision, need_dx, need_dw, False)
        if addend is not None and dx is not None:
            dx = dx + addend
        return dx, dw, db, dgamma, dbeta, dres
    args, dx, dw, dres, small, _keep = _layer_bwd_args(da, saved, rb, precision, training, relu, has_res, has_bias, need_dx,
                                                       need_dw, addend)
    cout = y.shape[1]
    L = _C.lib()
    if gsums is None:
        _C.check(L.toda_layer_bwd(ctypes.byref(args), _stream()), "toda_layer_bwd")
    else:
        red = torch.empty((2 * cout,), dtype=torch.float64, device=y.device)
        _C.check(L.toda_layer_bwd_reduce(ctypes.byref(args), _p(red), _stream()), "toda_layer_bwd_reduce")
        yield red
        _C.check(L.toda_layer_bwd_finish(ctypes.byref(args), _p(red), gsums.data_ptr() + 16 * cout, _stream()),
                 "toda_layer_bwd_finish")
    return dx, dw, (small[2 * cout:] if has_bias else None), small[:cout], small[cout:2 * cout], dres


def _layer_bwd_args(da, saved, rb, precision, training, relu, has_res, has_bias, need_dx, need_dw, addend):
    x, xb, weight, y, a_mask, gamma, mean, rstd, _ = saved
    L = _C.lib()
    da = da.contiguous()
    n_out, cout = y.shape
    cin, kvol, dev = weight.shape[4], rb.kvol, y.device
    bf16 = precision == CONV_BF16
    dy = torch.empty_like(y)
    dyb = torch.empty(y.shape, dtype=torch.bfloat16, device=dev) if bf16 else None
    dres = torch.empty_like(y) if has_res else None
    small = torch.empty((3 * cout,), dtype=torch.float32, device=dev)
    bws = _workspace("bn", L.toda_bn_workspace_bytes(cout), dev)
    dx = dw = None
    wt = wtb = None
    nbr = out_rows = masks = pl = None
    if need_dx:
        tc = bool(L.toda_spconv_uses_tensor_cores(cout, cin, kvol, precision))
        if tc and precision == CONV_BF16:
            wt, wtb = _repack(weight, True, rb.subm, True)
        else:
            wt = _repack(weight, True, rb.subm)
        if rb.subm:
            nbr, masks, pl = rb.nbr_fwd, rb.tile_masks, rb.plan
        elif rb.dgrad_order is None:
            nbr, pl = rb.nbr_bwd, rb.dgrad_plan
        else:
            nbr, out_rows, masks, pl = rb.nbr_bwd_sorted, rb.dgrad_order, rb.dgrad_tile_masks, rb.dgrad_plan
        if precision not in _TC_PRECISIONS:
            pl = None
        dx = torch.empty((rb.n_in, cin), dtype=torch.float32, device=dev)
        if addend is not None:
            addend = addend.contiguous()
    ws_bytes = L.toda_spconv_fwd_workspace_bytes(n_out, cout, cin, kvol, precision) if need_dx else 0
    ws = _workspace("conv", ws_bytes, dev) if ws_bytes else None
    wws = None
    if need_dw:
        dw = torch.empty_like(weight)
        wws = _workspace("wgrad", L.toda_spconv_wgrad_workspace_bytes(rb.n_in, n_out, kvol, cin, cout, precision), dev)
    sp = small.data_ptr()
    args = _C.LayerBwdArgs(
        da.data_ptr(), a_mask.data_ptr(), y.data_ptr(), n_out, cout, gamma.data_ptr(), _vp(mean), _vp(rstd), int(relu), int(training),
        dy.data_ptr(), _vp(dyb), _vp(dres), sp, sp + 4 * cout, bws.data_ptr(), bws.numel(),
        x.data_ptr(), _vp(xb), rb.n_in, cin, kvol,
        int(bool(need_dx)), _vp(nbr), _vp(wt), _vp(wtb), _vp(out_rows), _vp(masks),
        _vp(pl.lidx) if pl else None, _vp(pl.rows) if pl else None, _vp(pl.cnt) if pl else None, pl.ngroups if pl else 0,
        pl.cap if pl else 0, _vp(addend) if need_dx else None, _vp(dx),
        int(bool(need_dw)), rb.nbr_fwd.data_ptr(), _vp(rb.tile_masks), _vp(dw), _vp(wws), wws.numel() if wws is not None else 0,
        int(bool(has_bias)), sp + 8 * cout, precision, _vp(ws), ws.numel() if ws is not None else 0)
    return args, dx, dw, dres, small, (da, dy, dyb, addend, wt, wtb, ws, wws, bws)


class _ConvBNAct(torch.autograd.Function):

    @staticmethod
    def forward(ctx, x, x_bf16, weight, bias, rb, precision, gamma, beta, running_mean, running_var, eps, momentum, training,
                residual, relu, want_bf16, group):
        need_grad = any(ctx.needs_input_grad)
        a, ab, saved = _layer_forward(x, x_bf16, weight, bias, rb, precision, gamma, beta, running_mean, running_var, eps, momentum,
                                      training, residual, relu, want_bf16, need_grad, group)
        if need_grad:
            ctx.save_for_backward(*saved)
        ctx.set_materialize_grads(False)
        ctx.rb, ctx.precision, ctx.has_bias, ctx.group = rb, precision, bias is not None, group
        ctx.cfg = (bool(training), bool(relu), residual is not None, bool(want_bf16))
        if ab is not None:
            ctx.mark_non_differentiable(ab)
        return a, ab

    @staticmethod
    def backward(ctx, da, _dab=None):
        if da is None and ctx.group is None:
            return (None,) * 17
        training, relu, has_res, want_bf16 = ctx.cfg
        dx, dw, db, dgamma, dbeta, dres = _layer_backward(da, ctx.saved_tensors, ctx.rb, ctx.precision, training, relu, has_res,
                                                          ctx.has_bias and ctx.needs_input_grad[3], ctx.needs_input_grad[0],
                                                          ctx.needs_input_grad[2], group=ctx.group)
        return dx, None, dw, db, None, None, dgamma, dbeta, None, None, None, None, None, dres, None, None, None


class _ResBlock(torch.autograd.Function):

    @staticmethod
    def forward(ctx, x, x_bf16, w1, b1, g1, be1, rm1, rv1, w2, b2, g2, be2, rm2, rv2, rb, precision, eps, momentum, training, want_bf16,
                group1, group2):
        need_grad = any(ctx.needs_input_grad)
        h, hb, s1 = _layer_forward(x, x_bf16, w1, b1, rb, precision, g1, be1, rm1, rv1, eps, momentum, training, None, True,
                                   want_bf16, need_grad, group1)
        out, outb, s2 = _layer_forward(h, hb, w2, b2, rb, precision, g2, be2, rm2, rv2, eps, momentum, training, s1[0], True,
                                       want_bf16, need_grad, group2)
        if need_grad:
            ctx.save_for_backward(*s1, *s2)
        ctx.set_materialize_grads(False)
        ctx.rb, ctx.precision, ctx.training = rb, precision, bool(training)
        ctx.groups = (group1, group2)
        ctx.has_bias = (b1 is not None, b2 is not None)
        if outb is not None:
            ctx.mark_non_differentiable(outb)
        return out, outb

    @staticmethod
    def backward(ctx, dout, _db=None):
        if dout is None and ctx.groups == (None, None):
            return (None,) * 22
        sv = ctx.saved_tensors
        s1, s2 = sv[:9], sv[9:]
        ng = ctx.needs_input_grad
        dh, dw2, db2, dg2, dbe2, dres = _layer_backward(dout, s2, ctx.rb, ctx.precision, ctx.training, True, True,
                                                        ctx.has_bias[1] and ng[9], True, ng[8], group=ctx.groups[1])
        dx, dw1, db1, dg1, dbe1, _ = _layer_backward(dh, s1, ctx.rb, ctx.precision, ctx.training, True, False,
                                                     ctx.has_bias[0] and ng[3], ng[0], ng[2], addend=dres if ng[0] else None,
                                                     group=ctx.groups[0])
        return (dx, None, dw1, db1, dg1, dbe1, None, None, dw2, db2, dg2, dbe2, None, None, None, None, None, None, None, None,
                None, None)


def _bn_call(bn):
    group = sync_group(bn)
    training = bn.training or bn.running_mean is None
    if training and bn.running_mean is not None and bn.num_batches_tracked is not None:
        bn.num_batches_tracked += 1
    return training, group


def res_block(x, x_bf16, conv1_w, conv1_b, bn1, conv2_w, conv2_b, bn2, rb, precision, want_bf16=False):
    (training, group1), (training2, group2) = _bn_call(bn1), _bn_call(bn2)
    assert bn1.eps == bn2.eps and bn1.momentum == bn2.momentum and training == training2
    return _ResBlock.apply(x, x_bf16, conv1_w, conv1_b, bn1.weight, bn1.bias, bn1.running_mean, bn1.running_var, conv2_w, conv2_b,
                           bn2.weight, bn2.bias, bn2.running_mean, bn2.running_var, rb, precision, bn1.eps, bn1.momentum, training,
                           want_bf16, group1, group2)


def conv_bn_act(x, weight, bias, rb, precision, bn: torch.nn.BatchNorm1d, residual=None, relu=True, x_bf16=None, want_bf16=False):
    training, group = _bn_call(bn)
    return _ConvBNAct.apply(x, x_bf16, weight, bias, rb, precision, bn.weight, bn.bias, bn.running_mean, bn.running_var, bn.eps,
                            bn.momentum, training, residual, relu, want_bf16, group)


def bn_act(y, bn: torch.nn.BatchNorm1d, residual=None, relu=True, want_bf16=False, sums=None):
    training, group = _bn_call(bn)
    a, ab = _BNAct.apply(y, bn.weight, bn.bias, bn.running_mean, bn.running_var, bn.eps, bn.momentum, training, residual,
                         relu, want_bf16, sums if training else None, group)
    return (a, ab) if want_bf16 else a


class _BEVScatter(torch.autograd.Function):
    @staticmethod
    def forward(ctx, features, coords, batch, d, h, w):
        features = _need(features.contiguous(), torch.float32, "features")
        coords = _need(coords, torch.int32, "indices")
        n, c = features.shape
        out = torch.empty((batch, c * d, h, w), dtype=torch.float32, device=features.device)
        with _timed("bev_scatter_fwd", n=n, c=c, out_elems=out.numel()):
            _C.check(_C.lib().toda_bev_scatter_fwd(_p(features), _p(coords), n, c, batch, d, h, w, _p(out), _stream()),
                     "toda_bev_scatter_fwd")
        ctx.save_for_backward(coords)
        ctx.dims = (n, c, batch, d, h, w)
        return out

    @staticmethod
    def backward(ctx, dout):
        (coords,) = ctx.saved_tensors
        n, c, batch, d, h, w = ctx.dims
        dout = dout.contiguous()
        df = torch.empty((n, c), dtype=torch.float32, device=dout.device)
        with _timed("bev_scatter_bwd", n=n, c=c):
            _C.check(_C.lib().toda_bev_scatter_bwd(_p(dout), _p(coords), n, c, batch, d, h, w, _p(df), _stream()),
                     "toda_bev_scatter_bwd")
        return df, None, None, None, None, None


def bev_scatter(features, coords, batch, d, h, w):
    return _BEVScatter.apply(features, coords, batch, d, h, w)


class _GatherRows(torch.autograd.Function):
    @staticmethod
    def forward(ctx, x, rows, inverse_rows):
        x = _need(x.contiguous(), torch.float32, "features")
        n, c = rows.shape[0], x.shape[1]
        out = torch.empty((n, c), dtype=torch.float32, device=x.device)
        _C.check(_C.lib().toda_gather_rows(_p(x), _p(rows), n, c, _p(out), _stream()), "toda_gather_rows")
        ctx.save_for_backward(inverse_rows)
        return out

    @staticmethod
    def backward(ctx, dout):
        (inv,) = ctx.saved_tensors
        dout = dout.contiguous()
        n, c = inv.shape[0], dout.shape[1]
        dx = torch.empty((n, c), dtype=torch.float32, device=dout.device)
        _C.check(_C.lib().toda_gather_rows(_p(dout), _p(inv), n, c, _p(dx), _stream()), "toda_gather_rows")
        return dx, None, None


def permute_rows(x, rows, inverse_rows):
    return _GatherRows.apply(x, rows, inverse_rows)
```

Measured before the change: 419.9.

## Store ReLU masks as packed bits instead of rereading activations in BN backward

The BN apply kernel now emits a packed bitmask of positive outputs (1 bit per element via warp shuffles or ballot), and the BN backward reduce/finish kernels read these bits instead of the full fp32 activation tensor to gate gradients. This cuts backward memory traffic for the ReLU mask from 4 bytes to 1 bit per element. It adds extra shuffle/ballot work and bit-store traffic in forward, changes the C API and saved-tensor layout, and bumps the MODE 1 reduce unroll to 8.

Measured after the change: 424.4 (median of 6 runs). +1.1%, better.

```diff
diff --git a/include/toda_b200.h b/include/toda_b200.h
--- a/include/toda_b200.h
+++ b/include/toda_b200.h
@@ -107,19 +107,20 @@
 int toda_bn_eval_coeffs(const float *gamma, const float *beta, const float *running_mean, const float *running_var,
                         float eps, int channels, float *scale, float *shift, void *stream);
 int toda_bn_apply(const float *y, int n, int channels, const float *scale, const float *shift, const float *residual,
-                  int relu, float *a, void *a_bf16, void *stream);
+                  int relu, float *a, void *a_bf16, uint32_t *relu_bits, void *stream);
 int toda_bn_apply_sums(const float *y, int n, int channels, const double *sums, const double *count, const float *gamma,
                        const float *beta, float eps, float momentum, float *running_mean, float *running_var, float *scale,
                        float *shift, float *save_mean, float *save_rstd, const float *residual, int relu, float *a,
-                       void *a_bf16, void *stream);
-int toda_bn_bwd_reduce(const float *da, const float *a, const float *y, int n, int channels, const float *save_mean,
+                       void *a_bf16, uint32_t *relu_bits, void *stream);
+int toda_relu_bits(const float *a, long long total, uint32_t *bits, void *stream);
+int toda_bn_bwd_reduce(const float *da, const uint32_t *relu_bits, const float *y, int n, int channels, const float *save_mean,
                        const float *save_rstd, int relu, double *red, float *dgamma, float *dbeta, void *workspace,
                        size_t workspace_bytes, void *stream);
-int toda_bn_bwd_finish(const float *da, const float *a, const float *y, int n, int channels, const float *gamma,
+int toda_bn_bwd_finish(const float *da, const uint32_t *relu_bits, const float *y, int n, int channels, const float *gamma,
                        const float *save_mean, const float *save_rstd, int relu, int training, const double *red,
                        const double *count, float *dy, void *dy_bf16, float *dresidual, float *dbias, void *workspace,
                        size_t workspace_bytes, void *stream);
-int toda_bn_bwd(const float *da, const float *a, const float *y, int n, int channels, const float *gamma,
+int toda_bn_bwd(const float *da, const uint32_t *relu_bits, const float *y, int n, int channels, const float *gamma,
                 const float *save_mean, const float *save_rstd, int relu, int training, float *dy, void *dy_bf16,
                 float *dresidual, float *dgamma, float *dbeta, float *dbias, void *workspace, size_t workspace_bytes,
                 void *stream);
@@ -134,11 +135,11 @@
     int precision; void *conv_ws; size_t conv_ws_bytes;
     const float *gamma; const float *beta; float eps, momentum; float *running_mean; float *running_var; int training;
     const float *residual ; int relu;
-    float *y; double *sums; float *stats; float *a; void *a_bf16 ;
+    float *y; double *sums; float *stats; float *a; void *a_bf16 ; uint32_t *relu_bits ;
     void *bn_ws; size_t bn_ws_bytes;
 } toda_layer_fwd_args;
 typedef struct {
-    const float *da; const float *a_mask; const float *y; int n_out, cout; const float *gamma; const float *mean; const float *rstd;
+    const float *da; const uint32_t *relu_bits; const float *y; int n_out, cout; const float *gamma; const float *mean; const float *rstd;
     int relu, training; float *dy; void *dy_bf16 ; float *dres ; float *dgamma; float *dbeta;
     void *bn_ws; size_t bn_ws_bytes;
     const float *x; const void *x_bf16 ; int n_in, cin, kvol;
diff --git a/toda_b200/_C.py b/toda_b200/_C.py
--- a/toda_b200/_C.py
+++ b/toda_b200/_C.py
@@ -58,9 +58,10 @@
     "toda_bn_workspace_bytes": (c_sz, [c_int]),
     "toda_bn_local_sums": (c_int, [c_vp, c_vp, c_int, c_int, c_vp, c_vp, c_vp, c_sz, c_vp]),
     "toda_bn_eval_coeffs": (c_int, [c_vp, c_vp, c_vp, c_vp, c_f32, c_int, c_vp, c_vp, c_vp]),
-    "toda_bn_apply": (c_int, [c_vp, c_int, c_int, c_vp, c_vp, c_vp, c_int, c_vp, c_vp, c_vp]),
+    "toda_bn_apply": (c_int, [c_vp, c_int, c_int, c_vp, c_vp, c_vp, c_int, c_vp, c_vp, c_vp, c_vp]),
     "toda_bn_apply_sums": (c_int, [c_vp, c_int, c_int, c_vp, c_vp, c_vp, c_vp, c_f32, c_f32, c_vp, c_vp, c_vp, c_vp, c_vp, c_vp,
-                                   c_vp, c_int, c_vp, c_vp, c_vp]),
+                                   c_vp, c_int, c_vp, c_vp, c_vp, c_vp]),
+    "toda_relu_bits": (c_int, [c_vp, ctypes.c_longlong, c_vp, c_vp]),
     "toda_bn_bwd": (c_int, [c_vp, c_vp, c_vp, c_int, c_int, c_vp, c_vp, c_vp, c_int, c_int, c_vp, c_vp, c_vp, c_vp, c_vp,
                             c_vp, c_vp, c_sz, c_vp]),
     "toda_bn_bwd_reduce": (c_int, [c_vp, c_vp, c_vp, c_int, c_int, c_vp, c_vp, c_int, c_vp, c_vp, c_vp, c_vp, c_sz, c_vp]),
@@ -81,11 +82,12 @@
                 ("precision", c_int), ("conv_ws", c_vp), ("conv_ws_bytes", c_sz),
                 ("gamma", c_vp), ("beta", c_vp), ("eps", c_f32), ("momentum", c_f32), ("running_mean", c_vp), ("running_var", c_vp),
                 ("training", c_int), ("residual", c_vp), ("relu", c_int),
-                ("y", c_vp), ("sums", c_vp), ("stats", c_vp), ("a", c_vp), ("a_bf16", c_vp), ("bn_ws", c_vp), ("bn_ws_bytes", c_sz)]
+                ("y", c_vp), ("sums", c_vp), ("stats", c_vp), ("a", c_vp), ("a_bf16", c_vp), ("relu_bits", c_vp),
+                ("bn_ws", c_vp), ("bn_ws_bytes", c_sz)]
 
 
 class LayerBwdArgs(ctypes.Structure):
-    _fields_ = [("da", c_vp), ("a_mask", c_vp), ("y", c_vp), ("n_out", c_int), ("cout", c_int), ("gamma", c_vp), ("mean", c_vp),
+    _fields_ = [("da", c_vp), ("relu_bits", c_vp), ("y", c_vp), ("n_out", c_int), ("cout", c_int), ("gamma", c_vp), ("mean", c_vp),
                 ("rstd", c_vp), ("relu", c_int), ("training", c_int), ("dy", c_vp), ("dy_bf16", c_vp), ("dres", c_vp), ("dgamma", c_vp),
                 ("dbeta", c_vp), ("bn_ws", c_vp), ("bn_ws_bytes", c_sz),
                 ("x", c_vp), ("x_bf16", c_vp), ("n_in", c_int), ("cin", c_int), ("kvol", c_int),
diff --git a/toda_b200/csrc/bn.cu b/toda_b200/csrc/bn.cu
--- a/toda_b200/csrc/bn.cu
+++ b/toda_b200/csrc/bn.cu
@@ -8,8 +8,32 @@
 constexpr int kPartials = 2 * kNumSMs;
 constexpr int kApplyPartials = 2048 / kThreads * kNumSMs;
 
+
+__device__ __forceinline__ void relu_bits_pack4(uint32_t *__restrict__ bits, long long e, float4 o, bool valid) {
+    uint32_t w = valid ? (uint32_t)(o.x > 0.f) | (uint32_t)(o.y > 0.f) << 1 | (uint32_t)(o.z > 0.f) << 2 | (uint32_t)(o.w > 0.f) << 3
+                       : 0u;
+    w <<= (threadIdx.x & 7) * 4;
+    w |= __shfl_xor_sync(0xffffffffu, w, 1);
+    w |= __shfl_xor_sync(0xffffffffu, w, 2);
+    w |= __shfl_xor_sync(0xffffffffu, w, 4);
+    if ((threadIdx.x & 7) == 0 && valid) bits[e >> 3] = w;
+}
+
+__device__ __forceinline__ void relu_bits_pack1(uint32_t *__restrict__ bits, long long e, float o, bool valid) {
+    const uint32_t w = __ballot_sync(0xffffffffu, valid && o > 0.f);
+    if ((threadIdx.x & 31) == 0 && valid) bits[e >> 5] = w;
+}
+
+__device__ __forceinline__ uint32_t relu_nibble(const uint32_t *__restrict__ bits, long long e) {
+    return __ldg(bits + (e >> 3)) >> (((int)e & 7) * 4);
+}
+__device__ __forceinline__ bool relu_bit(const uint32_t *__restrict__ bits, long long e) {
+    return (__ldg(bits + (e >> 5)) >> ((int)e & 31)) & 1u;
+}
+
 template <int MODE>
-__global__ void __launch_bounds__(kThreads) col_reduce_vec_kernel(const float *__restrict__ p0, const float *__restrict__ p1,
+__global__ void __launch_bounds__(kThreads) col_reduce_vec_kernel(const float *__restrict__ p0,
+                                                                  const uint32_t *__restrict__ relu_bits,
                                                                   const float *__restrict__ p2, int n, int c,
                                                                   const float *__restrict__ mean, const float *__restrict__ rstd,
                                                                   int relu, double *__restrict__ partial) {
@@ -22,9 +46,10 @@
     if (MODE == 1) { m4 = __ldg((const float4 *)mean + tx); r4 = __ldg((const float4 *)rstd + tx); }
     const long long stride = (long long)gridDim.x * rpi;
     const bool active = ty < rpi;
-    constexpr int U = 4;
+    constexpr int U = MODE == 1 ? 8 : 4;
     for (long long r = (long long)blockIdx.x * rpi + ty; active && r < n; r += U * stride) {
-        float4 v0[U], v1[U], v2[U];
+        float4 v0[U], v2[U];
+        uint32_t m[U];
         bool ok[U];
 #pragma unroll
         for (int u = 0; u < U; ++u) {
@@ -32,7 +57,7 @@
             ok[u] = rr < n;
             size_t e = ok[u] ? (size_t)rr * tpr + tx : 0;
             v0[u] = __ldg((const float4 *)p0 + e);
-            if (MODE == 1) { v1[u] = __ldg((const float4 *)p1 + e); v2[u] = __ldg((const float4 *)p2 + e); }
+            if (MODE == 1) { m[u] = relu ? relu_nibble(relu_bits, e) : 0xFu; v2[u] = __ldg((const float4 *)p2 + e); }
         }
 #pragma unroll
         for (int u = 0; u < U; ++u) {
@@ -42,11 +67,11 @@
 #pragma unroll
                 for (int q = 0; q < 4; ++q) { a0[q] += x[q]; a1[q] += (double)x[q] * x[q]; }
             } else if (MODE == 1) {
-                float av[4] = {v1[u].x, v1[u].y, v1[u].z, v1[u].w}, yv[4] = {v2[u].x, v2[u].y, v2[u].z, v2[u].w};
+                float yv[4] = {v2[u].x, v2[u].y, v2[u].z, v2[u].w};
                 float mm[4] = {m4.x, m4.y, m4.z, m4.w}, rs[4] = {r4.x, r4.y, r4.z, r4.w};
 #pragma unroll
                 for (int q = 0; q < 4; ++q) {
-                    float g = (relu && !(av[q] > 0.f)) ? 0.f : x[q];
+                    float g = (m[u] >> q) & 1u ? x[q] : 0.f;
                     float xh = (yv[q] - mm[q]) * rs[q];
                     a0[q] += g; a1[q] += (double)g * xh;
                 }
@@ -69,7 +94,7 @@
 }
 
 template <int MODE>
-__global__ void __launch_bounds__(kThreads) col_reduce_kernel(const float *__restrict__ p0, const float *__restrict__ p1,
+__global__ void __launch_bounds__(kThreads) col_reduce_kernel(const float *__restrict__ p0, const uint32_t *__restrict__ relu_bits,
                                                               const float *__restrict__ p2, int n, int c,
                                                               const float *__restrict__ mean, const float *__restrict__ rstd,
                                                               int relu, double *__restrict__ partial) {
@@ -88,7 +113,7 @@
                 a0 += v; a1 += (double)v * v;
             } else if (MODE == 1) {
                 float g = __ldg(p0 + e);
-                if (relu && !(__ldg(p1 + e) > 0.f)) g = 0.f;
+                if (relu && !relu_bit(relu_bits, e)) g = 0.f;
                 float xh = (__ldg(p2 + e) - m) * rs;
                 a0 += g; a1 += (double)g * xh;
             } else {
@@ -109,12 +134,12 @@
 static bool vec_channels(int c) { return c % 4 == 0 && kThreads % (c / 4) == 0; }
 
 template <int MODE>
-static void launch_col_reduce(const float *p0, const float *p1, const float *p2, int n, int c, const float *mean,
+static void launch_col_reduce(const float *p0, const uint32_t *relu_bits, const float *p2, int n, int c, const float *mean,
                               const float *rstd, int relu, double *partial, cudaStream_t st) {
     if (vec_channels(c))
-        col_reduce_vec_kernel<MODE><<<kPartials, kThreads, 0, st>>>(p0, p1, p2, n, c, mean, rstd, relu, partial);
+        col_reduce_vec_kernel<MODE><<<kPartials, kThreads, 0, st>>>(p0, relu_bits, p2, n, c, mean, rstd, relu, partial);
     else
-        col_reduce_kernel<MODE><<<kPartials, kThreads, 0, st>>>(p0, p1, p2, n, c, mean, rstd, relu, partial);
+        col_reduce_kernel<MODE><<<kPartials, kThreads, 0, st>>>(p0, relu_bits, p2, n, c, mean, rstd, relu, partial);
 }
 
 template <int MAX_BLOCKS = kPartials, int ROWS = 2>
@@ -195,10 +220,10 @@
     float *running_mean, *running_var, *scale, *shift, *save_mean, *save_rstd;
 };
 
-template <bool VEC>
+template <bool VEC, bool BITS>
 __global__ void __launch_bounds__(kThreads) bn_apply_kernel(const float *__restrict__ y, long long total, int c, BnCoeffs k,
                                                             const float *__restrict__ residual, int relu, float *__restrict__ a,
-                                                            __nv_bfloat16 *__restrict__ a_bf16) {
+                                                            __nv_bfloat16 *__restrict__ a_bf16, uint32_t *__restrict__ relu_bits) {
     extern __shared__ __align__(16) float s_coef[];
     float *s_sc = s_coef, *s_sh = s_coef + c;
     const int n = k.count ? (int)*k.count : k.n;
@@ -222,12 +247,13 @@
     }
     __syncthreads();
     const long long stride = (long long)gridDim.x * blockDim.x;
+    const int lane = threadIdx.x & 31;
     long long e = blockIdx.x * (long long)blockDim.x + threadIdx.x;
     if (VEC) {
         const long long tv = total >> 2;
         const int ch = (int)((e << 2) % c);
         const float4 sc = *(const float4 *)(s_sc + ch), sh = *(const float4 *)(s_sh + ch);
-        for (; e < tv; e += stride) {
+        auto apply = [&](long long e) {
             const float4 v = __ldg((const float4 *)y + e);
             float4 o = make_float4(fmaf(v.x, sc.x, sh.x), fmaf(v.y, sc.y, sh.y), fmaf(v.z, sc.z, sh.z), fmaf(v.w, sc.w, sh.w));
             if (residual) {
@@ -237,16 +263,39 @@
             if (relu) { o.x = fmaxf(o.x, 0.f); o.y = fmaxf(o.y, 0.f); o.z = fmaxf(o.z, 0.f); o.w = fmaxf(o.w, 0.f); }
             ((float4 *)a)[e] = o;
             if (a_bf16) store_bf16x4(a_bf16, e, o);
-        }
+            return o;
+        };
+        if (!BITS) {
+            for (; e < tv; e += stride) apply(e);
+            return;
+        }
+        for (; e - lane + 32 <= tv; e += stride) relu_bits_pack4(relu_bits, e, apply(e), true);
+        if (e - lane < tv) relu_bits_pack4(relu_bits, e, e < tv ? apply(e) : make_float4(0.f, 0.f, 0.f, 0.f), e < tv);
     } else {
-        for (; e < total; e += stride) {
-            const int ch = (int)(e % c);
-            float o = fmaf(__ldg(y + e), s_sc[ch], s_sh[ch]);
+        auto apply = [&](long long e) {
+            float o = fmaf(__ldg(y + e), s_sc[(int)(e % c)], s_sh[(int)(e % c)]);
             if (residual) o += __ldg(residual + e);
             if (relu) o = fmaxf(o, 0.f);
             a[e] = o;
             if (a_bf16) a_bf16[e] = __float2bfloat16_rn(o);
-        }
+            return o;
+        };
+        if (!BITS) {
+            for (; e < total; e += stride) apply(e);
+            return;
+        }
+        for (; e - lane + 32 <= total; e += stride) relu_bits_pack1(relu_bits, e, apply(e), true);
+        if (e - lane < total) relu_bits_pack1(relu_bits, e, e < total ? apply(e) : 0.f, e < total);
+    }
+}
+
+__global__ void __launch_bounds__(kThreads) relu_bits_kernel(const float *__restrict__ a, long long total,
+                                                             uint32_t *__restrict__ bits) {
+    const long long stride = (long long)gridDim.x * blockDim.x;
+    const int lane = threadIdx.x & 31;
+    for (long long e = blockIdx.x * (long long)blockDim.x + threadIdx.x; e - lane < total; e += stride) {
+        const bool ok = e < total;
+        relu_bits_pack1(bits, e, ok ? __ldg(a + e) : 0.f, ok);
     }
 }
 
@@ -264,7 +313,8 @@
 }
 
 template <bool VEC>
-__global__ void __launch_bounds__(kThreads, 5) bn_bwd_apply_kernel(const float *__restrict__ da, const float *__restrict__ a,
+__global__ void __launch_bounds__(kThreads, 5) bn_bwd_apply_kernel(const float *__restrict__ da,
+                                                                const uint32_t *__restrict__ relu_bits,
                                                                 const float *__restrict__ y, long long total, int c, int n,
                                                                 const double *__restrict__ count, const float *__restrict__ gamma,
                                                                 const float *__restrict__ mean, const float *__restrict__ rstd,
@@ -290,13 +340,14 @@
             B[q] = training ? -gm * rs * rs * sum(c + ch + q) * inv_n : 0.f;
             C[q] = training ? -A[q] * sum(ch + q) * inv_n - B[q] * mean[ch + q] : 0.f;
         }
+        const int mshift = (threadIdx.x & 7) * 4;
         for (; e < tv; e += stride) {
             float4 g4 = __ldg((const float4 *)da + e);
             float4 y4 = training ? __ldg((const float4 *)y + e) : make_float4(0.f, 0.f, 0.f, 0.f);
             if (relu) {
-                float4 a4 = __ldg((const float4 *)a + e);
-                g4.x = a4.x > 0.f ? g4.x : 0.f; g4.y = a4.y > 0.f ? g4.y : 0.f;
-                g4.z = a4.z > 0.f ? g4.z : 0.f; g4.w = a4.w > 0.f ? g4.w : 0.f;
+                const uint32_t m = __ldg(relu_bits + (e >> 3)) >> mshift;
+                g4.x = m & 1u ? g4.x : 0.f; g4.y = m & 2u ? g4.y : 0.f;
+                g4.z = m & 4u ? g4.z : 0.f; g4.w = m & 8u ? g4.w : 0.f;
             }
             if (dres) ((float4 *)dres)[e] = g4;
             float4 o;
@@ -312,7 +363,7 @@
         for (e = e < stride ? e : total; e < total; e += stride) {
             int ch = (int)(e % c);
             float g = __ldg(da + e);
-            if (relu && !(__ldg(a + e) > 0.f)) g = 0.f;
+            if (relu && !relu_bit(relu_bits, e)) g = 0.f;
             if (dres) dres[e] = g;
             float gm = gamma ? gamma[ch] : 1.f;
             float rs = rstd[ch];
@@ -367,16 +418,24 @@
     return (int)(need < 1 ? 1 : (need < cap ? need : cap));
 }
 
+template <bool VEC, bool BITS>
+void launch_bn_apply_kernel(const float *y, long long total, int c, const BnCoeffs &k, const float *residual, int relu, float *a,
+                            void *a_bf16, uint32_t *relu_bits, cudaStream_t st) {
+    bn_apply_kernel<VEC, BITS><<<resident_grid<bn_apply_kernel<VEC, BITS>>(VEC ? total / 4 : total), kThreads,
+                                 2 * (size_t)c * sizeof(float), st>>>(y, total, c, k, residual, relu, a, (__nv_bfloat16 *)a_bf16,
+                                                                      relu_bits);
+}
+
 int launch_bn_apply(const float *y, int n, int c, const BnCoeffs &k, const float *residual, int relu, float *a, void *a_bf16,
-                    cudaStream_t st) {
+                    uint32_t *relu_bits, cudaStream_t st) {
     const long long total = (long long)n * c;
-    const size_t smem = 2 * (size_t)c * sizeof(float);
+    const bool bits = relu && relu_bits;
     if (vec_channels(c))
-        bn_apply_kernel<true><<<resident_grid<bn_apply_kernel<true>>(total / 4), kThreads, smem, st>>>(
-            y, total, c, k, residual, relu, a, (__nv_bfloat16 *)a_bf16);
+        (bits ? launch_bn_apply_kernel<true, true> : launch_bn_apply_kernel<true, false>)(y, total, c, k, residual, relu, a, a_bf16,
+                                                                                          relu_bits, st);
     else
-        bn_apply_kernel<false><<<resident_grid<bn_apply_kernel<false>>(total), kThreads, smem, st>>>(
-            y, total, c, k, residual, relu, a, (__nv_bfloat16 *)a_bf16);
+        (bits ? launch_bn_apply_kernel<false, true> : launch_bn_apply_kernel<false, false>)(y, total, c, k, residual, relu, a,
+                                                                                            a_bf16, relu_bits, st);
     TODA_LAUNCH_OK();
     return TODA_OK;
 }
@@ -416,49 +475,57 @@
 }
 
 extern "C" int toda_bn_apply(const float *y, int n, int c, const float *scale, const float *shift, const float *residual,
-                             int relu, float *a, void *a_bf16, void *stream) {
+                             int relu, float *a, void *a_bf16, uint32_t *relu_bits, void *stream) {
     TODA_CHECK_ARG(n >= 0 && c > 0, "bn_apply: bad sizes");
     if (n == 0) return TODA_OK;
     TODA_CHECK_ARG(y && scale && shift && a, "bn_apply: null pointer");
     BnCoeffs k{};
     k.scale = (float *)scale;
     k.shift = (float *)shift;
-    return launch_bn_apply(y, n, c, k, residual, relu, a, a_bf16, (cudaStream_t)stream);
+    return launch_bn_apply(y, n, c, k, residual, relu, a, a_bf16, relu_bits, (cudaStream_t)stream);
 }
 
 extern "C" int toda_bn_apply_sums(const float *y, int n, int c, const double *sums, const double *count, const float *gamma,
                                   const float *beta, float eps, float momentum, float *running_mean, float *running_var,
                                   float *scale, float *shift, float *save_mean, float *save_rstd, const float *residual, int relu,
-                                  float *a, void *a_bf16, void *stream) {
+                                  float *a, void *a_bf16, uint32_t *relu_bits, void *stream) {
     TODA_CHECK_ARG(n >= 0 && c > 0 && sums && scale && shift, "bn_apply_sums: bad args");
     TODA_CHECK_ARG(n == 0 || (y && a), "bn_apply_sums: null pointer");
     const BnCoeffs k{sums, count, n, gamma, beta, eps, momentum, running_mean, running_var, scale, shift, save_mean, save_rstd};
-    return launch_bn_apply(y, n, c, k, residual, relu, a, a_bf16, (cudaStream_t)stream);
-}
-
-extern "C" int toda_bn_bwd_reduce(const float *da, const float *a, const float *y, int n, int c, const float *save_mean,
+    return launch_bn_apply(y, n, c, k, residual, relu, a, a_bf16, relu_bits, (cudaStream_t)stream);
+}
+
+extern "C" int toda_relu_bits(const float *a, long long total, uint32_t *bits, void *stream) {
+    TODA_CHECK_ARG(total >= 0 && (total == 0 || (a && bits)), "relu_bits: bad args");
+    if (total == 0) return TODA_OK;
+    relu_bits_kernel<<<resident_grid<relu_bits_kernel>(total), kThreads, 0, (cudaStream_t)stream>>>(a, total, bits);
+    TODA_LAUNCH_OK();
+    return TODA_OK;
+}
+
+extern "C" int toda_bn_bwd_reduce(const float *da, const uint32_t *relu_bits, const float *y, int n, int c, const float *save_mean,
                                   const float *save_rstd, int relu, double *local_red, float *dgamma, float *dbeta, void *workspace,
                                   size_t workspace_bytes, void *stream) {
     TODA_CHECK_ARG(n >= 0 && c > 0 && c <= 256, "bn_bwd_reduce: unsupported sizes n=%d c=%d", n, c);
-    TODA_CHECK_ARG(save_mean && save_rstd && workspace && local_red && (n == 0 || (da && y)) && (!relu || a || n == 0),
+    TODA_CHECK_ARG(save_mean && save_rstd && workspace && local_red && (n == 0 || (da && y)) && (!relu || relu_bits || n == 0),
                    "bn_bwd_reduce: null pointer");
     if (workspace_bytes < bn_ws_bytes(c)) { toda_set_error("bn_bwd_reduce: workspace too small"); return TODA_ERR_WORKSPACE; }
     cudaStream_t st = (cudaStream_t)stream;
     double *partial = (double *)workspace;
-    launch_col_reduce<1>(da, a, y, n, c, save_mean, save_rstd, relu, partial, st);
+    launch_col_reduce<1>(da, relu_bits, y, n, c, save_mean, save_rstd, relu, partial, st);
     TODA_LAUNCH_OK();
     bn_bwd_finalize_kernel<<<ceil_div(c * 32, 128), 128, 0, st>>>(partial, kPartials, c, dgamma, dbeta, local_red);
     TODA_LAUNCH_OK();
     return TODA_OK;
 }
 
-extern "C" int toda_bn_bwd_finish(const float *da, const float *a, const float *y, int n, int c, const float *gamma,
+extern "C" int toda_bn_bwd_finish(const float *da, const uint32_t *relu_bits, const float *y, int n, int c, const float *gamma,
                                   const float *save_mean, const float *save_rstd, int relu, int training, const double *red,
                                   const double *count, float *dy, void *dy_bf16, float *dresidual, float *dbias, void *workspace,
                                   size_t workspace_bytes, void *stream) {
     TODA_CHECK_ARG(n >= 0 && c > 0 && c <= 256, "bn_bwd_finish: unsupported sizes n=%d c=%d", n, c);
     TODA_CHECK_ARG(save_mean && save_rstd && (red || !training) && (n == 0 || (da && y && (dy || dy_bf16))) &&
-                   (!relu || a || n == 0) && (!dbias || workspace), "bn_bwd_finish: null pointer");
+                   (!relu || relu_bits || n == 0) && (!dbias || workspace), "bn_bwd_finish: null pointer");
     cudaStream_t st = (cudaStream_t)stream;
     if (dbias && workspace_bytes < bn_ws_bytes(c)) { toda_set_error("bn_bwd_finish: workspace too small"); return TODA_ERR_WORKSPACE; }
     if (n == 0) {
@@ -472,12 +539,12 @@
     if (vec_channels(c)) {
         grid = resident_grid<bn_bwd_apply_kernel<true>>(total / 4);
         grid = grid < kApplyPartials ? grid : kApplyPartials;
-        bn_bwd_apply_kernel<true><<<grid, kThreads, smem, st>>>(da, a, y, total, c, n, count, gamma, save_mean, save_rstd, red, relu,
+        bn_bwd_apply_kernel<true><<<grid, kThreads, smem, st>>>(da, relu_bits, y, total, c, n, count, gamma, save_mean, save_rstd, red, relu,
                                                                training, dy, dresidual, (__nv_bfloat16 *)dy_bf16, db_partial);
     } else {
         grid = resident_grid<bn_bwd_apply_kernel<false>>(total);
         grid = grid < kApplyPartials ? grid : kApplyPartials;
-        bn_bwd_apply_kernel<false><<<grid, kThreads, smem, st>>>(da, a, y, total, c, n, count, gamma, save_mean, save_rstd, red,
+        bn_bwd_apply_kernel<false><<<grid, kThreads, smem, st>>>(da, relu_bits, y, total, c, n, count, gamma, save_mean, save_rstd, red,
                                                                 relu, training, dy, dresidual, (__nv_bfloat16 *)dy_bf16, db_partial);
     }
     TODA_LAUNCH_OK();
@@ -488,15 +555,15 @@
     return TODA_OK;
 }
 
-extern "C" int toda_bn_bwd(const float *da, const float *a, const float *y, int n, int c, const float *gamma,
+extern "C" int toda_bn_bwd(const float *da, const uint32_t *relu_bits, const float *y, int n, int c, const float *gamma,
                            const float *save_mean, const float *save_rstd, int relu, int training, float *dy, void *dy_bf16,
                            float *dresidual, float *dgamma, float *dbeta, float *dbias, void *workspace, size_t workspace_bytes,
                            void *stream) {
     TODA_CHECK_ARG(workspace, "bn_bwd: null workspace");
     double *red = bn_workspace_red(workspace, c);
-    int rc = toda_bn_bwd_reduce(da, a, y, n, c, save_mean, save_rstd, relu, red, dgamma, dbeta, workspace, workspace_bytes, stream);
+    int rc = toda_bn_bwd_reduce(da, relu_bits, y, n, c, save_mean, save_rstd, relu, red, dgamma, dbeta, workspace, workspace_bytes, stream);
     if (rc) return rc;
-    return toda_bn_bwd_finish(da, a, y, n, c, gamma, save_mean, save_rstd, relu, training, red, nullptr, dy, dy_bf16, dresidual,
+    return toda_bn_bwd_finish(da, relu_bits, y, n, c, gamma, save_mean, save_rstd, relu, training, red, nullptr, dy, dy_bf16, dresidual,
                               dbias, workspace, workspace_bytes, stream);
 }
 
diff --git a/toda_b200/csrc/layer.cu b/toda_b200/csrc/layer.cu
--- a/toda_b200/csrc/layer.cu
+++ b/toda_b200/csrc/layer.cu
@@ -18,7 +18,7 @@
     const int c = p->cout;
     float *scale = p->stats, *shift = p->stats + c, *mean = p->stats + 2 * c, *rstd = p->stats + 3 * c;
     return toda_bn_apply_sums(p->y, p->n_out, c, sums, count, p->gamma, p->beta, p->eps, p->momentum, p->running_mean,
-                              p->running_var, scale, shift, mean, rstd, p->residual, p->relu, p->a, p->a_bf16, stream);
+                              p->running_var, scale, shift, mean, rstd, p->residual, p->relu, p->a, p->a_bf16, p->relu_bits, stream);
 }
 
 extern "C" int toda_layer_fwd(const toda_layer_fwd_args *p, void *stream) {
@@ -35,7 +35,7 @@
     float *scale = p->stats, *shift = p->stats + c;
     if ((rc = layer_conv(p, nullptr, stream))) return rc;
     if ((rc = toda_bn_eval_coeffs(p->gamma, p->beta, p->running_mean, p->running_var, p->eps, c, scale, shift, stream))) return rc;
-    return toda_bn_apply(p->y, n, c, scale, shift, p->residual, p->relu, p->a, p->a_bf16, stream);
+    return toda_bn_apply(p->y, n, c, scale, shift, p->residual, p->relu, p->a, p->a_bf16, p->relu_bits, stream);
 }
 
 static int layer_bwd_empty(const toda_layer_bwd_args *p, bool bn_grads, cudaStream_t st) {
@@ -76,14 +76,14 @@
 }
 
 static int layer_bwd_reduce(const toda_layer_bwd_args *p, double *red, void *stream) {
-    return toda_bn_bwd_reduce(p->da, p->a_mask, p->y, p->n_out, p->cout, p->mean, p->rstd, p->relu, red, p->dgamma, p->dbeta,
+    return toda_bn_bwd_reduce(p->da, p->relu_bits, p->y, p->n_out, p->cout, p->mean, p->rstd, p->relu, red, p->dgamma, p->dbeta,
                               p->bn_ws, p->bn_ws_bytes, stream);
 }
 
 static int layer_bwd_finish(const toda_layer_bwd_args *p, const double *red, const double *count, void *stream) {
     const int c = p->cout, n = p->n_out;
     if (n == 0) return layer_bwd_empty(p, false, (cudaStream_t)stream);
-    int rc = toda_bn_bwd_finish(p->da, p->a_mask, p->y, n, c, p->gamma, p->mean, p->rstd, p->relu, p->training, red, count,
+    int rc = toda_bn_bwd_finish(p->da, p->relu_bits, p->y, n, c, p->gamma, p->mean, p->rstd, p->relu, p->training, red, count,
                                 layer_bwd_reads_dy_f32(p) ? p->dy : nullptr, p->dy_bf16, p->dres, p->need_db ? p->db : nullptr,
                                 p->bn_ws, p->bn_ws_bytes, stream);
     return rc ? rc : layer_bwd_conv(p, stream);
diff --git a/toda_b200/ops.py b/toda_b200/ops.py
--- a/toda_b200/ops.py
+++ b/toda_b200/ops.py
@@ -662,6 +662,21 @@
     _relu_tape = tape
 
 
+def relu_bits(a):
+    a = _need(a.contiguous(), torch.float32, "activation")
+    bits = _relu_bits_buffer(a.numel(), a.device)
+    _C.check(_C.lib().toda_relu_bits(_p(a), a.numel(), _p(bits), _stream()), "toda_relu_bits")
+    return bits
+
+
+def _relu_bits_buffer(elements, device):
+    return torch.empty(((elements + 31) // 32,), dtype=torch.int32, device=device)
+
+
+def _as_relu_bits(mask):
+    return relu_bits(mask) if mask.dtype == torch.float32 else mask
+
+
 def sync_group(bn):
     if not isinstance(bn, torch.nn.SyncBatchNorm) or not bn.training:
         return None
@@ -696,7 +711,7 @@
 
 
 def _bn_forward_phases(y, gamma, beta, running_mean, running_var, eps, momentum, training, residual, relu, want_bf16, sums,
-                       need_grad, sync=False):
+                       need_grad, sync=False, want_bits=True):
     y = _need(y.contiguous(), torch.float32, "bn input")
     n, c = y.shape
     dev = y.device
@@ -725,22 +740,26 @@
     tape = _relu_tape is not None and relu
     ab = torch.empty(y.shape, dtype=torch.bfloat16, device=dev) if (want_bf16 and not tape) else None
     act = 0 if tape else int(relu)
+    want_bits = want_bits and need_grad
+    bits = _relu_bits_buffer(n * c, dev) if (act and want_bits) else None
     with _timed("bn_apply", n=n, c=c, residual=res is not None):
         if training:
             _C.check(L.toda_bn_apply_sums(_p(y), n, c, _p(sums), count, _p(gamma), _p(beta), float(eps), float(momentum),
                                           _p(running_mean), _p(running_var), _p(scale), _p(shift), _p(mean), _p(rstd), _p(res),
-                                          act, _p(a), _p(ab), _stream()), "toda_bn_apply_sums")
+                                          act, _p(a), _p(ab), _p(bits), _stream()), "toda_bn_apply_sums")
         else:
-            _C.check(L.toda_bn_apply(_p(y), n, c, _p(scale), _p(shift), _p(res), act, _p(a), _p(ab), _stream()), "toda_bn_apply")
+            _C.check(L.toda_bn_apply(_p(y), n, c, _p(scale), _p(shift), _p(res), act, _p(a), _p(ab), _p(bits), _stream()),
+                     "toda_bn_apply")
     if tape:
         a, ab, mask = _tape_mask(a, want_bf16)
-        return a, ab, y, mean, rstd, mask, gsums
-    return a, ab, y, mean, rstd, a, gsums
+        bits = relu_bits(mask) if want_bits else None
+    return a, ab, y, mean, rstd, bits, gsums
 
 
 def _bn_backward_phases(da, y, a, gamma, mean, rstd, training, relu, has_res, want_bf16, gsums=None, want_db=False):
     n, c = y.shape
     da = da.contiguous() if da is not None else torch.zeros_like(y)
+    bits = _as_relu_bits(a) if relu else None
     L = _C.lib()
     dy = torch.empty_like(y)
     dyb = torch.empty(y.shape, dtype=torch.bfloat16, device=y.device) if want_bf16 else None
@@ -750,15 +769,15 @@
     ws = _workspace("bn", L.toda_bn_workspace_bytes(c), y.device)
     if gsums is None:
         with _timed("bn_bwd", n=n, c=c, residual=has_res):
-            _C.check(L.toda_bn_bwd(_p(da), _p(a), _p(y), n, c, _p(gamma), _p(mean), _p(rstd), int(relu), int(training),
+            _C.check(L.toda_bn_bwd(_p(da), _p(bits), _p(y), n, c, _p(gamma), _p(mean), _p(rstd), int(relu), int(training),
                                    _p(dy), _p(dyb), _p(dres), _p(dgamma), _p(dbeta), _p(db), _p(ws), ws.numel(), _stream()),
                      "toda_bn_bwd")
         return dy, dyb, dres, dgamma, dbeta, db
     red = torch.empty((2 * c,), dtype=torch.float64, device=y.device)
-    _C.check(L.toda_bn_bwd_reduce(_p(da), _p(a), _p(y), n, c, _p(mean), _p(rstd), int(relu), _p(red), _p(dgamma), _p(dbeta),
+    _C.check(L.toda_bn_bwd_reduce(_p(da), _p(bits), _p(y), n, c, _p(mean), _p(rstd), int(relu), _p(red), _p(dgamma), _p(dbeta),
                                   _p(ws), ws.numel(), _stream()), "toda_bn_bwd_reduce")
     yield red
-    _C.check(L.toda_bn_bwd_finish(_p(da), _p(a), _p(y), n, c, _p(gamma), _p(mean), _p(rstd), int(relu), 1, _p(red),
+    _C.check(L.toda_bn_bwd_finish(_p(da), _p(bits), _p(y), n, c, _p(gamma), _p(mean), _p(rstd), int(relu), 1, _p(red),
                                   gsums.data_ptr() + 16 * c, _p(dy), _p(dyb), _p(dres), _p(db), _p(ws), ws.numel(), _stream()),
              "toda_bn_bwd_finish")
     return dy, dyb, dres, dgamma, dbeta, db
@@ -766,11 +785,12 @@
 
 class _BNAct(torch.autograd.Function):
     @staticmethod
-    def forward(ctx, y, gamma, beta, running_mean, running_var, eps, momentum, training, residual, relu, want_bf16, sums, group):
-        a, ab, y, mean, rstd, a_mask, gsums = _run_phases(
+    def forward(ctx, y, gamma, beta, running_mean, running_var, eps, momentum, training, residual, relu, want_bf16, sums, group,
+                grad_mode):
+        a, ab, y, mean, rstd, bits, gsums = _run_phases(
             _bn_forward_phases(y, gamma, beta, running_mean, running_var, eps, momentum, training, residual, relu, want_bf16, sums,
-                        y.requires_grad or gamma.requires_grad, group is not None), group)
-        ctx.save_for_backward(y, a_mask, gamma, mean, rstd, gsums)
+                        any(ctx.needs_input_grad), group is not None, grad_mode), group)
+        ctx.save_for_backward(y, bits, gamma, mean, rstd, gsums)
         ctx.set_materialize_grads(False)
         ctx.cfg = (bool(training), bool(relu), residual is not None, bool(want_bf16))
         ctx.group = group
@@ -781,14 +801,14 @@
     @staticmethod
     def backward(ctx, da, _dab=None):
         if da is None and ctx.group is None:
-            return (None,) * 13
-        y, a, gamma, mean, rstd, gsums = ctx.saved_tensors
+            return (None,) * 14
+        y, bits, gamma, mean, rstd, gsums = ctx.saved_tensors
         training, relu, has_res, want_bf16 = ctx.cfg
-        dy, dyb, dres, dgamma, dbeta, _ = _run_phases(_bn_backward_phases(da, y, a, gamma, mean, rstd, training, relu, has_res,
+        dy, dyb, dres, dgamma, dbeta, _ = _run_phases(_bn_backward_phases(da, y, bits, gamma, mean, rstd, training, relu, has_res,
                                                                           want_bf16, gsums), ctx.group)
         if dyb is not None:
             dy._toda_bf16 = (dyb, dy._version)
-        return dy, dgamma, dbeta, None, None, None, None, None, dres, None, None, None, None
+        return dy, dgamma, dbeta, None, None, None, None, None, dres, None, None, None, None, None
 
 
 def _vp(t):
@@ -800,22 +820,23 @@
 
 
 def _layer_forward(x, x_bf16, weight, bias, rb, precision, gamma, beta, running_mean, running_var, eps, momentum, training,
-                   residual, relu, want_bf16, need_grad=True, group=None):
+                   residual, relu, want_bf16, need_grad=True, group=None, want_bits=True):
     return _run_phases(_layer_forward_phases(x, x_bf16, weight, bias, rb, precision, gamma, beta, running_mean, running_var, eps,
-                                             momentum, residual, relu, want_bf16, need_grad, training, group is not None), group)
+                                             momentum, residual, relu, want_bf16, need_grad, training, group is not None, want_bits),
+                       group)
 
 
 def _layer_forward_phases(x, x_bf16, weight, bias, rb, precision, gamma, beta, running_mean, running_var, eps, momentum,
-                          residual, relu, want_bf16, need_grad=True, training=True, sync=True):
+                          residual, relu, want_bf16, need_grad=True, training=True, sync=True, want_bits=True):
     if not _fused_ok(training, need_grad):
         y, sums, x, weight, x_bf16 = _conv_forward_impl(x, x_bf16, weight, bias, rb, precision, bool(training))
-        a, ab, y, mean, rstd, a_mask, gsums = yield from _bn_forward_phases(y, gamma, beta, running_mean, running_var, eps,
-                                                                            momentum, training, residual, relu, want_bf16, sums,
-                                                                            need_grad, sync)
-        return a, ab, (x, x_bf16, weight, y, a_mask, gamma, mean, rstd, gsums)
-    args, x, x_bf16, weight, y, a, ab, small, _keep = _layer_fwd_args(
+        a, ab, y, mean, rstd, bits, gsums = yield from _bn_forward_phases(y, gamma, beta, running_mean, running_var, eps,
+                                                                          momentum, training, residual, relu, want_bf16, sums,
+                                                                          need_grad, sync, want_bits)
+        return a, ab, (x, x_bf16, weight, y, a, gamma, mean, rstd, gsums, bits)
+    args, x, x_bf16, weight, y, a, ab, bits, small, _keep = _layer_fwd_args(
         x, x_bf16, weight, bias, rb, precision, gamma, beta, running_mean, running_var, eps, momentum, training, residual, relu,
-        want_bf16)
+        want_bf16, need_grad and want_bits)
     cout = y.shape[1]
     L = _C.lib()
     gsums = None
@@ -828,11 +849,11 @@
         _C.check(L.toda_layer_fwd(ctypes.byref(args), _stream()), "toda_layer_fwd")
     mean = small[2 * cout:3 * cout] if training else running_mean
     rstd = small[3 * cout:4 * cout] if training else None
-    return a, ab, (x, x_bf16, weight, y, a, gamma, mean, rstd, gsums)
+    return a, ab, (x, x_bf16, weight, y, a, gamma, mean, rstd, gsums, bits)
 
 
 def _layer_fwd_args(x, x_bf16, weight, bias, rb, precision, gamma, beta, running_mean, running_var, eps, momentum, training,
-                    residual, relu, want_bf16):
+                    residual, relu, want_bf16, want_bits):
     x = _need(x.contiguous(), torch.float32, "features")
     weight = _need(weight.contiguous(), torch.float32, "weight")
     cout, cin = weight.shape[0], weight.shape[4]
@@ -850,6 +871,7 @@
     y = torch.empty((n_out, cout), dtype=torch.float32, device=dev)
     a = torch.empty_like(y)
     ab = torch.empty((n_out, cout), dtype=torch.bfloat16, device=dev) if want_bf16 else None
+    bits = _relu_bits_buffer(n_out * cout, dev) if (relu and want_bits) else None
     small = torch.empty((8 * cout,), dtype=torch.float32, device=dev)
     ws_bytes = L.toda_spconv_fwd_workspace_bytes(x.shape[0], cin, cout, kvol, precision)
     ws = _workspace("conv", ws_bytes, dev) if ws_bytes else None
@@ -863,8 +885,9 @@
         _vp(rb.tile_masks), _vp(pl.lidx) if pl else None, _vp(pl.rows) if pl else None, _vp(pl.cnt) if pl else None,
         pl.ngroups if pl else 0, pl.cap if pl else 0, precision, _vp(ws), ws.numel() if ws is not None else 0,
         gamma.data_ptr(), beta.data_ptr(), float(eps), float(momentum), _vp(running_mean), _vp(running_var), int(bool(training)),
-        _vp(res), int(bool(relu)), y.data_ptr(), sp + 16 * cout, sp, a.data_ptr(), _vp(ab), bws.data_ptr(), bws.numel())
-    return args, x, x_bf16, weight, y, a, ab, small, (w, wb, ws, bws, res, b)
+        _vp(res), int(bool(relu)), y.data_ptr(), sp + 16 * cout, sp, a.data_ptr(), _vp(ab), _vp(bits), bws.data_ptr(),
+        bws.numel())
+    return args, x, x_bf16, weight, y, a, ab, bits, small, (w, wb, ws, bws, res, b)
 
 
 def _layer_backward(da, saved, rb, precision, training, relu, has_res, has_bias, need_dx, need_dw, addend=None, group=None):
@@ -873,11 +896,11 @@
 
 
 def _layer_backward_phases(da, saved, rb, precision, relu, has_res, has_bias, need_dx, need_dw, addend=None, training=True):
-    x, xb, weight, y, a_mask, gamma, mean, rstd, gsums = saved
+    x, xb, weight, y, _, gamma, mean, rstd, gsums, bits = saved
     if da is None:
         da = torch.zeros_like(y)
     if not _fused_ok(training, True):
-        dy, dyb, dres, dgamma, dbeta, db = yield from _bn_backward_phases(da, y, a_mask, gamma, mean, rstd, training, relu,
+        dy, dyb, dres, dgamma, dbeta, db = yield from _bn_backward_phases(da, y, bits, gamma, mean, rstd, training, relu,
                                                                           has_res, precision == CONV_BF16, gsums, has_bias)
         dx, dw, _ = _conv_backward_impl(dy, dyb, x, weight, xb, rb, precision, need_dx, need_dw, False)
         if addend is not None and dx is not None:
@@ -899,7 +922,8 @@
 
 
 def _layer_bwd_args(da, saved, rb, precision, training, relu, has_res, has_bias, need_dx, need_dw, addend):
-    x, xb, weight, y, a_mask, gamma, mean, rstd, _ = saved
+    x, xb, weight, y, _, gamma, mean, rstd, _, bits = saved
+    bits = _as_relu_bits(bits) if relu else None
     L = _C.lib()
     da = da.contiguous()
     n_out, cout = y.shape
@@ -938,7 +962,7 @@
         wws = _workspace("wgrad", L.toda_spconv_wgrad_workspace_bytes(rb.n_in, n_out, kvol, cin, cout, precision), dev)
     sp = small.data_ptr()
     args = _C.LayerBwdArgs(
-        da.data_ptr(), a_mask.data_ptr(), y.data_ptr(), n_out, cout, gamma.data_ptr(), _vp(mean), _vp(rstd), int(relu), int(training),
+        da.data_ptr(), _vp(bits), y.data_ptr(), n_out, cout, gamma.data_ptr(), _vp(mean), _vp(rstd), int(relu), int(training),
         dy.data_ptr(), _vp(dyb), _vp(dres), sp, sp + 4 * cout, bws.data_ptr(), bws.numel(),
         x.data_ptr(), _vp(xb), rb.n_in, cin, kvol,
         int(bool(need_dx)), _vp(nbr), _vp(wt), _vp(wtb), _vp(out_rows), _vp(masks),
@@ -946,17 +970,17 @@
         pl.cap if pl else 0, _vp(addend) if need_dx else None, _vp(dx),
         int(bool(need_dw)), rb.nbr_fwd.data_ptr(), _vp(rb.tile_masks), _vp(dw), _vp(wws), wws.numel() if wws is not None else 0,
         int(bool(has_bias)), sp + 8 * cout, precision, _vp(ws), ws.numel() if ws is not None else 0)
-    return args, dx, dw, dres, small, (da, dy, dyb, addend, wt, wtb, ws, wws, bws)
+    return args, dx, dw, dres, small, (da, bits, dy, dyb, addend, wt, wtb, ws, wws, bws)
 
 
 class _ConvBNAct(torch.autograd.Function):
 
     @staticmethod
     def forward(ctx, x, x_bf16, weight, bias, rb, precision, gamma, beta, running_mean, running_var, eps, momentum, training,
-                residual, relu, want_bf16, group):
+                residual, relu, want_bf16, group, grad_mode):
         need_grad = any(ctx.needs_input_grad)
         a, ab, saved = _layer_forward(x, x_bf16, weight, bias, rb, precision, gamma, beta, running_mean, running_var, eps, momentum,
-                                      training, residual, relu, want_bf16, need_grad, group)
+                                      training, residual, relu, want_bf16, need_grad, group, grad_mode)
         if need_grad:
             ctx.save_for_backward(*saved)
         ctx.set_materialize_grads(False)
@@ -969,24 +993,24 @@
     @staticmethod
     def backward(ctx, da, _dab=None):
         if da is None and ctx.group is None:
-            return (None,) * 17
+            return (None,) * 18
         training, relu, has_res, want_bf16 = ctx.cfg
         dx, dw, db, dgamma, dbeta, dres = _layer_backward(da, ctx.saved_tensors, ctx.rb, ctx.precision, training, relu, has_res,
                                                           ctx.has_bias and ctx.needs_input_grad[3], ctx.needs_input_grad[0],
                                                           ctx.needs_input_grad[2], group=ctx.group)
-        return dx, None, dw, db, None, None, dgamma, dbeta, None, None, None, None, None, dres, None, None, None
+        return dx, None, dw, db, None, None, dgamma, dbeta, None, None, None, None, None, dres, None, None, None, None
 
 
 class _ResBlock(torch.autograd.Function):
 
     @staticmethod
     def forward(ctx, x, x_bf16, w1, b1, g1, be1, rm1, rv1, w2, b2, g2, be2, rm2, rv2, rb, precision, eps, momentum, training, want_bf16,
-                group1, group2):
+                group1, group2, grad_mode):
         need_grad = any(ctx.needs_input_grad)
         h, hb, s1 = _layer_forward(x, x_bf16, w1, b1, rb, precision, g1, be1, rm1, rv1, eps, momentum, training, None, True,
-                                   want_bf16, need_grad, group1)
+                                   want_bf16, need_grad, group1, grad_mode)
         out, outb, s2 = _layer_forward(h, hb, w2, b2, rb, precision, g2, be2, rm2, rv2, eps, momentum, training, s1[0], True,
-                                       want_bf16, need_grad, group2)
+                                       want_bf16, need_grad, group2, grad_mode)
         if need_grad:
             ctx.save_for_backward(*s1, *s2)
         ctx.set_materialize_grads(False)
@@ -1000,9 +1024,9 @@
     @staticmethod
     def backward(ctx, dout, _db=None):
         if dout is None and ctx.groups == (None, None):
-            return (None,) * 22
+            return (None,) * 23
         sv = ctx.saved_tensors
-        s1, s2 = sv[:9], sv[9:]
+        s1, s2 = sv[:len(sv) // 2], sv[len(sv) // 2:]
         ng = ctx.needs_input_grad
         dh, dw2, db2, dg2, dbe2, dres = _layer_backward(dout, s2, ctx.rb, ctx.precision, ctx.training, True, True,
                                                         ctx.has_bias[1] and ng[9], True, ng[8], group=ctx.groups[1])
@@ -1010,7 +1034,7 @@
                                                      ctx.has_bias[0] and ng[3], ng[0], ng[2], addend=dres if ng[0] else None,
                                                      group=ctx.groups[0])
         return (dx, None, dw1, db1, dg1, dbe1, None, None, dw2, db2, dg2, dbe2, None, None, None, None, None, None, None, None,
-                None, None)
+                None, None, None)
 
 
 def _bn_call(bn):
@@ -1026,19 +1050,19 @@
     assert bn1.eps == bn2.eps and bn1.momentum == bn2.momentum and training == training2
     return _ResBlock.apply(x, x_bf16, conv1_w, conv1_b, bn1.weight, bn1.bias, bn1.running_mean, bn1.running_var, conv2_w, conv2_b,
                            bn2.weight, bn2.bias, bn2.running_mean, bn2.running_var, rb, precision, bn1.eps, bn1.momentum, training,
-                           want_bf16, group1, group2)
+                           want_bf16, group1, group2, torch.is_grad_enabled())
 
 
 def conv_bn_act(x, weight, bias, rb, precision, bn: torch.nn.BatchNorm1d, residual=None, relu=True, x_bf16=None, want_bf16=False):
     training, group = _bn_call(bn)
     return _ConvBNAct.apply(x, x_bf16, weight, bias, rb, precision, bn.weight, bn.bias, bn.running_mean, bn.running_var, bn.eps,
-                            bn.momentum, training, residual, relu, want_bf16, group)
+                            bn.momentum, training, residual, relu, want_bf16, group, torch.is_grad_enabled())
 
 
 def bn_act(y, bn: torch.nn.BatchNorm1d, residual=None, relu=True, want_bf16=False, sums=None):
     training, group = _bn_call(bn)
     a, ab = _BNAct.apply(y, bn.weight, bn.bias, bn.running_mean, bn.running_var, bn.eps, bn.momentum, training, residual,
-                         relu, want_bf16, sums if training else None, group)
+                         relu, want_bf16, sums if training else None, group, torch.is_grad_enabled())
     return (a, ab) if want_bf16 else a
 
 
```
